# pangsu0613/TransCAR

Measured on AMD Instinct MI355X. Metric: nuScenes frames/sec (6-cam+radar, 900 queries): fusion decoder (Detr3DHead.forward + box decode), FPN features resident in HBM, higher is better.
Workload: dtype f32 (linear steps and attention core of the batched launches: f16x2 split operands, 3 v_mfma_f32_16x16x32_f16 products, fp32 accumulate; activations of the 32-row tiles held as two f16 planes; 4- / 8-row tiles: f32 MFMA)

## Files before the change

### include/transcar_hip.h

```cpp
#ifndef TRANSCAR_HIP_H
#define TRANSCAR_HIP_H

#include <stddef.h>

#ifdef __cplusplus
extern "C" {
#endif

#define TC_MAX_LEVELS 4
#define TC_MAX_LAYERS 8
#define TC_MAX_RADAR_LAYERS 3
#define TC_MAX_CAM_LOGITS 256
#define TC_RADAR_HEADS 8
#define TC_MAX_CLASSES 32
#define TC_BOX_DECODE_MAX_SCORES 12288
#define TC_BOX_DECODE_MAX_NUM 512
#define TC_BOX_DECODE_STREAM_MAX_SCORES (1 << 20)
#define TC_BOX_DECODE_STREAM_MAX_NUM 2048
#define TC_LSA_MAX_QUERIES 4096
#define TC_LSA_MAX_GT 512
#define TC_LSA_SMALL_MAX_QUERIES 1024
#define TC_LSA_SMALL_MAX_GT 128
#define TC_LSA_AUTO 0
#define TC_LSA_SMALL 1
// ... 127 lines not shown

int tc_refine_reference_fwd(const float* reg_out, int code_size, const float* ref,
                            float* new_ref, int M, tc_stream_t stream);

int tc_cam_sample_fuse_fwd(const tc_feats_nhwc* feats, int B, int Q, int C, int num_cams,
                           const float* lidar2img , const float* ref ,
                           const float* attn_logits ,
                           const float* pc_range , float img_h, float img_w,
                           float* out, unsigned char* vis_mask,
                           unsigned long long* pair_counter ,
                           tc_stream_t stream);

int tc_cam_sample_fuse_points_fwd(const tc_feats_nhwc* feats, int B, int Q, int C, int num_cams, int num_points,
                                  const float* lidar2img , const float* ref ,
                                  const float* attn_logits ,
                                  const float* pc_range , float img_h, float img_w,
                                  float* out, unsigned char* vis_mask,
                                  unsigned long long* pair_counter ,
                                  tc_stream_t stream);

size_t tc_cross_atten_workspace_bytes(int B, int Q, int C, int num_cams, int num_levels);
int tc_cross_atten_fwd(const tc_linear* attention_weights, const tc_linear* output_proj,
                       const tc_pos_encoder* position_encoder,
                       const tc_feats_nhwc* feats, int B, int Q, int C, int num_cams,
                       const float* query, const float* query_pos,
                       const float* lidar2img, const float* ref,
                       const float* pc_range , float img_h, float img_w,
                       float* out, void* workspace, size_t workspace_bytes,
                       tc_stream_t stream);
size_t tc_cross_atten_points_workspace_bytes(int B, int Q, int C, int num_cams, int num_levels, int num_points);
int tc_cross_atten_points_fwd(const tc_linear* attention_weights, const tc_linear* output_proj,
                              const tc_pos_encoder* position_encoder,
                              const tc_feats_nhwc* feats, int B, int Q, int C, int num_cams, int num_points,
                              const float* query, const float* query_pos,
                              const float* lidar2img, const float* ref,
                              const float* pc_range , float img_h, float img_w,
                              float* out, void* workspace, size_t workspace_bytes,
                              tc_stream_t stream);

size_t tc_self_attn_workspace_bytes(int B, int Q, int C);
int tc_self_attn_fwd(const tc_mha* w, const float* x, const float* pos, float* out,
                     int B, int Q, int C, int num_heads,
                     void* workspace, size_t workspace_bytes, tc_stream_t stream);

int tc_decoder_layer_tail_fwd(const tc_decoder_layer* layer, const tc_linear* next_in_proj,
                              const tc_feats_nhwc* feats, int B, int Q, int num_cams,
                              int code_size, const float* attn_o, const float* x_in,
                              const float* query_embedding, const float* lidar2img,
                              const float* ref_in, const float* pc_range ,
                              float img_h, float img_w, float* hs, float* ref_out,
                              float* qk, float* vt, int qpad,
                              int tile_rows , tc_stream_t stream);

int tc_sdpa_fwd(const float* q, const float* k, int ld, const float* vt, int ldt,
                float* out, int ldo, int B, int Q, int num_heads, tc_stream_t stream);
size_t tc_sdpa_f16x2_workspace_bytes(int B, int Q, int num_heads);
int tc_sdpa_fwd_f16x2(const float* qk, const float* vt, int ldt, float* out, int ldo, int B, int Q, int num_heads,
                      void* workspace, size_t workspace_bytes, tc_stream_t stream);
int tc_sdpa_fwd_hd(const float* q, const float* k, int ld, const float* vt, int ldt,
                   float* out, int ldo, int B, int Q, int num_heads, int head_dim, tc_stream_t stream);
int tc_sdpa_fwd_f16x2_hd(const float* qk, const float* vt, int ldt, float* out, int ldo, int B, int Q, int num_heads,
                         int head_dim, tc_stream_t stream);

size_t tc_radar_xattn_workspace_bytes(int B, int Q, int T, int C);
int tc_radar_gated_xattn_fwd(const tc_mha* w, const float* query, const float* centre_xy,
                             const float* box, int code_size,
                             const float* radar_feat, const float* radar_xy,
                             int B, int Q, int T, int C, int num_heads, int pad_mult,
                             float radius_min, float radius_max,
                             float* out, int* hit_counts,
                             void* workspace, size_t workspace_bytes, tc_stream_t stream);

int tc_radar_fusion_fwd(const tc_head_weights* packed_view, const float* hs_last,
                        const float* ref_last, const float* prev_box, const float* radar_tokens,
                        int B, int T, int pad_mult, int first_layer, int num_layers,
                        float* all_cls_scores, float* all_bbox_preds, int* hit_counts,
                        const tc_head_options* options, void* workspace, size_t workspace_bytes,
                        tc_stream_t stream);

int tc_radar_gate_selfcheck(int n_radii, unsigned long long seed, unsigned long long* mismatches,
                            tc_stream_t stream);

int tc_rowops_selfcheck(int n_blocks, unsigned long long seed, unsigned long long* mismatches, tc_stream_t stream);

size_t tc_box_decode_workspace_bytes(int B, int Q, int num_classes);
int tc_box_decode_topk(const float* cls_scores ,
                       const float* bbox_preds , int B, int Q,
                       int num_classes, int code_size, int max_num,
                       const float* post_center_range ,
                       float* boxes, float* scores, int* labels, unsigned char* valid,
                       void* workspace, size_t workspace_bytes, tc_stream_t stream);
int tc_box_decode_kept(const float* cls_scores, const float* bbox_preds, int B, int Q, int num_classes,
                       int code_size, int max_num, const float* post_center_range ,
                       float score_threshold, int use_threshold, int z_shift,
                       float* kept_boxes, float* kept_scores, long long* kept_labels, int* kept_count,
                       tc_stream_t stream);
int tc_box_decode_topk_path(const float* cls_scores, const float* bbox_preds, int B, int Q,
                            int num_classes, int code_size, int max_num,
                            const float* post_center_range ,
                            float* boxes, float* scores, int* labels, unsigned char* valid,
                            void* workspace, size_t workspace_bytes, tc_stream_t stream, int path);
int tc_box_decode_kept_path(const float* cls_scores, const float* bbox_preds, int B, int Q, int num_classes,
                            int code_size, int max_num, const float* post_center_range ,
                            float score_threshold, int use_threshold, int z_shift,
                            float* kept_boxes, float* kept_scores, long long* kept_labels, int* kept_count,
                            tc_stream_t stream, int path);

size_t tc_head_workspace_bytes(const tc_head_weights* w, int B, int T);
size_t tc_cam_pregather_workspace_bytes(const tc_head_weights* w, int B);
size_t tc_head_packed_bytes(const tc_head_weights* w);
int tc_head_pack_weights(const tc_head_weights* w, void* packed, size_t packed_bytes,
                         tc_head_weights* packed_view, tc_stream_t stream);
int tc_head_repack_trainable(const tc_head_weights* w, tc_head_weights* packed_view,
                             tc_stream_t stream);
int tc_head_repack_trainable_ex(const tc_head_weights* w, tc_head_weights* packed_view, int copies,
                                tc_stream_t stream);
int tc_head_forward(const tc_head_weights* w, const tc_head_weights* packed_view,
                    const tc_feats_nhwc* feats, int B,
                    const float* lidar2img , float img_h, float img_w,
                    const float* radar_tokens, int T, int pad_mult,
                    float* all_cls_scores, float* all_bbox_preds,
                    const tc_head_aux* aux ,
                    const tc_head_options* options ,
                    void* workspace, size_t workspace_bytes, tc_stream_t stream);

typedef struct {
  int abi_version;
  int num_levels, embed_dims, num_classes, code_size;
  float pc_range[6];
  tc_cls_branch cls[TC_MAX_LAYERS];
  tc_reg_branch reg[TC_MAX_LAYERS];
  size_t packed16_delta;
} tc_decoder_heads;
size_t tc_decoder_heads_packed_bytes(const tc_decoder_heads* w);
int tc_decoder_heads_pack(const tc_decoder_heads* w, void* packed, size_t packed_bytes,
                          tc_decoder_heads* packed_view, tc_stream_t stream);
int tc_decoder_outputs_fwd(const tc_decoder_heads* packed_view,
                           const float* inter_states     ,
                           const float* init_reference   ,
                           const float* inter_references ,
                           int B, int Q,
                           float* all_cls_scores ,
                           float* all_bbox_preds ,
                           const tc_head_options* options , tc_stream_t stream);



int tc_linear_gated_fwd(const float* x, const float* w, const float* b, const float* res,
                        const int* row_gate, float* y, int M, int K, int N, tc_stream_t stream);

int tc_linear_bwd_data(const float* dy, const float* y_relu, const int* row_gate,
                       const float* w, const float* x_relu, float* dx, int M, int K, int N,
                       float alpha, int accumulate, tc_stream_t stream);
int tc_linear_bwd_weight(const float* x, const float* dy, const float* y_relu,
                         const int* row_gate, float* dw, float* db, int M, int K, int N,
                         float alpha, tc_stream_t stream);

int tc_add_layernorm_bwd(const float* a, const float* b, const float* gamma, const float* dy,
                         const float* y_relu, float* dz, float* dgamma, float* dbeta, int M,
                         int C, tc_stream_t stream);

int tc_radar_reference_l1(const float* ref, const float* pc_range , float* centre_xy,
                          float* add_ref, int M, tc_stream_t stream);

int tc_box_add_ref_fwd(const float* reg_out, int code_size, const float* ref_xy, int ld_xy,
                       const float* ref_z, int ld_z, float* box, int M, tc_stream_t stream);
// ... 102 lines not shown
```

### transcar_amd/_lib.py

```python
import ctypes as C
import os

import torch

_HERE = os.path.dirname(os.path.abspath(__file__))
LIB_PATH = os.environ.get('TRANSCAR_HIP_LIB') or os.path.join(_HERE, 'lib', 'libtranscar_hip.so')

TC_MAX_LEVELS = 4
TC_MAX_LAYERS = 8
TC_MAX_RADAR_LAYERS = 3
TC_ABI_VERSION = 13

c_fp = C.c_void_p


class TransCARHipError(RuntimeError):
    pass


TC_MAX_CAM_LOGITS = 256


def check_num_points(num_points, num_cams, num_levels):
    if int(num_points) < 1 or num_cams * num_levels * int(num_points) > TC_MAX_CAM_LOGITS:
# ... 127 lines not shown
                ('num_points', C.c_int)]


class tc_decoder_heads(C.Structure):
    _fields_ = [('abi_version', C.c_int), ('num_levels', C.c_int), ('embed_dims', C.c_int),
                ('num_classes', C.c_int), ('code_size', C.c_int),
                ('pc_range', C.c_float * 6),
                ('cls', tc_cls_branch * TC_MAX_LAYERS), ('reg', tc_reg_branch * TC_MAX_LAYERS),
                ('packed16_delta', C.c_size_t)]


class tc_feats_nhwc(C.Structure):
    _fields_ = [('num_levels', C.c_int),
                ('data', c_fp * TC_MAX_LEVELS),
                ('H', C.c_int * TC_MAX_LEVELS),
                ('W', C.c_int * TC_MAX_LEVELS)]


class tc_head_aux(C.Structure):
    _fields_ = [('inter_states', c_fp), ('init_reference', c_fp),
                ('inter_references', c_fp), ('radar_hit_counts', c_fp),
                ('last_box', c_fp), ('sample_pairs', c_fp)]


class tc_head_options(C.Structure):
    _fields_ = [('chain_tile_rows', C.c_int), ('unfused', C.c_int),
                ('last_level_cls_only', C.c_int), ('reuse_radar_kv', C.c_int),
                ('decoder_dropout_p', C.c_float), ('radar_row_order', C.c_int),
                ('dropout_seed', C.c_ulonglong), ('phase', C.c_int), ('matrix_path', C.c_int),
                ('dropout_seed_stride', C.c_ulonglong), ('range_status', c_fp), ('cam_pregather', C.c_int),
                ('cam_pregather_ws', c_fp), ('cam_pregather_bytes', C.c_size_t)]


TC_MATRIX_AUTO, TC_MATRIX_F32, TC_MATRIX_F16X2 = 0, 1, 2


_P = C.POINTER
_i, _f, _sz, _vp = C.c_int, C.c_float, C.c_size_t, C.c_void_p

SIGNATURES = {
    'tc_abi_version': (_i, []),
    'tc_last_error': (C.c_char_p, []),
    'tc_chain_tile_rows': (_i, [_i, _i, _i]),
    'tc_device_count': (_i, []),
    'tc_nchw_to_nhwc': (_i, [_vp, _vp, _i, _i, _i, _i, _vp]),
    'tc_nchw_to_nhwc_levels': (_i, [_P(_vp), _P(_vp), _i, _i, _i, _P(_i), _P(_i), _vp]),
    'tc_radar_build_tokens': (_i, [_vp, _vp, _P(_i), _i, _P(C.c_double), _P(C.c_double),
                                   _P(C.c_double), _vp, _i, _vp, _vp]),
    'tc_radar_build_tokens_batch': (_i, [_vp, _vp, _vp, _i, _i, _vp, _i, _vp, _vp]),
    'tc_linear_fwd': (_i, [_vp, _vp, _vp, _vp, _vp, _vp, _i, _i, _i, _i, _vp]),
    'tc_add_layernorm_fwd': (_i, [_vp, _vp, _vp, _vp, _vp, _i, _i, _i, _vp]),
    'tc_refine_reference_fwd': (_i, [_vp, _i, _vp, _vp, _i, _vp]),
    'tc_cam_sample_fuse_fwd': (_i, [_P(tc_feats_nhwc), _i, _i, _i, _i, _vp,
                                    _vp, _vp, _P(_f), _f, _f, _vp, _vp, _vp,
                                    _vp]),
    'tc_cam_sample_fuse_points_fwd': (_i, [_P(tc_feats_nhwc), _i, _i, _i, _i, _i,
                                           _vp, _vp, _vp, _P(_f), _f, _f, _vp,
                                           _vp, _vp, _vp]),
    'tc_cross_atten_workspace_bytes': (_sz, [_i, _i, _i, _i, _i]),
    'tc_cross_atten_points_workspace_bytes': (_sz, [_i, _i, _i, _i, _i, _i]),
    'tc_cross_atten_points_fwd': (_i, [_P(tc_linear), _P(tc_linear),
                                       _P(tc_pos_encoder), _P(tc_feats_nhwc),
                                       _i, _i, _i, _i, _i, _vp, _vp, _vp, _vp,
                                       _P(_f), _f, _f, _vp, _vp, _sz, _vp]),
    'tc_cross_atten_fwd': (_i, [_P(tc_linear), _P(tc_linear),
                                _P(tc_pos_encoder), _P(tc_feats_nhwc), _i, _i,
                                _i, _i, _vp, _vp, _vp, _vp, _P(_f), _f, _f,
                                _vp, _vp, _sz, _vp]),
    'tc_self_attn_workspace_bytes': (_sz, [_i, _i, _i]),
    'tc_self_attn_fwd': (_i, [_P(tc_mha), _vp, _vp, _vp, _i, _i, _i, _i, _vp,
                              _sz, _vp]),
    'tc_decoder_layer_tail_fwd': (_i, [_P(tc_decoder_layer), _P(tc_linear),
                                       _P(tc_feats_nhwc), _i, _i, _i, _i, _vp,
                                       _vp, _vp, _vp, _vp, _P(_f), _f, _f, _vp,
                                       _vp, _vp, _vp, _i, _i, _vp]),
    'tc_sdpa_fwd': (_i, [_vp, _vp, _i, _vp, _i, _vp, _i, _i, _i, _i, _vp]),
    'tc_sdpa_f16x2_workspace_bytes': (_sz, [_i, _i, _i]),
    'tc_sdpa_fwd_f16x2': (_i, [_vp, _vp, _i, _vp, _i, _i, _i, _i, _vp, _sz, _vp]),
    'tc_sdpa_fwd_hd': (_i, [_vp, _vp, _i, _vp, _i, _vp, _i, _i, _i, _i, _i, _vp]),
    'tc_sdpa_fwd_f16x2_hd': (_i, [_vp, _vp, _i, _vp, _i, _i, _i, _i, _i, _vp]),
    'tc_radar_xattn_workspace_bytes': (_sz, [_i, _i, _i, _i]),
    'tc_radar_gate_selfcheck': (_i, [_i, C.c_ulonglong, _vp, _vp]),
    'tc_rowops_selfcheck': (_i, [_i, C.c_ulonglong, _vp, _vp]),
    'tc_radar_gated_xattn_fwd': (_i, [_P(tc_mha), _vp, _vp, _vp, _i, _vp, _vp,
                                      _i, _i, _i, _i, _i, _i, _f, _f, _vp,
                                      _vp, _vp, _sz, _vp]),
    'tc_radar_fusion_fwd': (_i, [_P(tc_head_weights), _vp, _vp, _vp, _vp, _i, _i, _i, _i, _i,
                                 _vp, _vp, _vp, _P(tc_head_options), _vp, _sz, _vp]),
    'tc_box_decode_workspace_bytes': (_sz, [_i, _i, _i]),
    'tc_box_decode_topk': (_i, [_vp, _vp, _i, _i, _i, _i, _i, _P(_f), _vp,
                                _vp, _vp, _vp, _vp, _sz, _vp]),
    'tc_box_decode_kept': (_i, [_vp, _vp, _i, _i, _i, _i, _i, _P(_f), _f, _i, _i, _vp, _vp, _vp, _vp, _vp]),
    'tc_box_decode_topk_path': (_i, [_vp, _vp, _i, _i, _i, _i, _i, _P(_f), _vp,
                                     _vp, _vp, _vp, _vp, _sz, _vp, _i]),
    'tc_box_decode_kept_path': (_i, [_vp, _vp, _i, _i, _i, _i, _i, _P(_f), _f, _i, _i, _vp, _vp, _vp, _vp, _vp, _i]),
    'tc_head_workspace_bytes': (_sz, [_P(tc_head_weights), _i, _i]),
    'tc_cam_pregather_workspace_bytes': (_sz, [_P(tc_head_weights), _i]),
    'tc_head_packed_bytes': (_sz, [_P(tc_head_weights)]),
    'tc_head_pack_weights': (_i, [_P(tc_head_weights), _vp, _sz,
                                  _P(tc_head_weights), _vp]),
    'tc_head_repack_trainable': (_i, [_P(tc_head_weights), _P(tc_head_weights), _vp]),
    'tc_head_forward': (_i, [_P(tc_head_weights), _P(tc_head_weights),
                             _P(tc_feats_nhwc), _i, _vp,
                             _f, _f, _vp, _i, _i, _vp, _vp, _P(tc_head_aux),
                             _P(tc_head_options), _vp, _sz, _vp]),
    'tc_decoder_heads_packed_bytes': (_sz, [_P(tc_decoder_heads)]),
    'tc_decoder_heads_pack': (_i, [_P(tc_decoder_heads), _vp, _sz, _P(tc_decoder_heads), _vp]),
    'tc_decoder_outputs_fwd': (_i, [_P(tc_decoder_heads), _vp, _vp, _vp, _i, _i, _vp, _vp,
                                    _P(tc_head_options), _vp]),
    'tc_linear_gated_fwd': (_i, [_vp, _vp, _vp, _vp, _vp, _vp, _i, _i, _i, _vp]),
    'tc_linear_bwd_data': (_i, [_vp, _vp, _vp, _vp, _vp, _vp, _i, _i, _i, _f,
                                _i, _vp]),
    'tc_linear_bwd_weight': (_i, [_vp, _vp, _vp, _vp, _vp, _vp, _i, _i, _i, _f,
                                  _vp]),
    'tc_add_layernorm_bwd': (_i, [_vp, _vp, _vp, _vp, _vp, _vp, _vp, _vp, _i,
                                  _i, _vp]),
    'tc_radar_reference_l1': (_i, [_vp, _P(_f), _vp, _vp, _i, _vp]),
    'tc_box_add_ref_fwd': (_i, [_vp, _i, _vp, _i, _vp, _i, _vp, _i, _vp]),
    'tc_box_add_ref_bwd': (_i, [_vp, _i, _vp, _i, _vp]),
    'tc_radar_attn_core_fwd': (_i, [_vp, _f, _vp, _vp, _i, _vp, _i, _vp, _i,
                                    _i, _i, _i, _i, _i, _i, _f, _f, _vp, _vp,
                                    _f, C.c_ulonglong, _i, _vp]),
    'tc_dropout': (_i, [_vp, _i, _i, _f, C.c_ulonglong, _i, _vp, _vp]),
    'tc_radar_attn_core_bwd': (_i, [_vp, _f, _vp, _vp, _i, _vp, _i, _vp, _i,
                                    _i, _i, _i, _i, _i, _i, _f, _f, _vp, _vp,
                                    _vp, _vp, _f, C.c_ulonglong, _i, _vp]),
    'tc_radar_train_tape_bytes': (_sz, [_P(tc_head_weights), _i, _i]),
    'tc_radar_train_fwd': (_i, [_P(tc_head_weights), _vp, _vp, _vp, _vp, _i, _i,
                                _i, _vp, _vp, _vp, _sz, _f, C.c_ulonglong, _vp]),
    'tc_radar_train_fwd_fused': (_i, [_P(tc_head_weights), _vp, _vp, _vp, _vp, _i, _i,
                                      _i, _vp, _vp, _vp, _sz, _f, C.c_ulonglong, _vp]),
    'tc_head_repack_trainable_ex': (_i, [_P(tc_head_weights), _P(tc_head_weights), _i, _vp]),
    'tc_radar_train_bwd': (_i, [_P(tc_head_weights), _P(tc_head_weights), _vp,
                                _vp, _vp, _i, _i, _i, _vp, _vp, _vp, _vp, _sz,
                                _f, C.c_ulonglong, _vp]),
    'tc_radar_train_bwd_workspace_bytes': (_sz, [_P(tc_head_weights), _i, _i]),
    'tc_radar_train_bwd_fused': (_i, [_P(tc_head_weights), _P(tc_head_weights), _vp,
                                      _vp, _vp, _i, _i, _i, _vp, _vp, _vp, _vp, _sz, _vp, _sz,
                                      _f, C.c_ulonglong, _vp, _vp, _vp]),
    'tc_radar_train_bwd_fused_ex': (_i, [_P(tc_head_weights), _P(tc_head_weights), _vp,
                                         _vp, _vp, _i, _i, _i, _vp, _vp, _vp, _vp, _sz, _vp, _sz,
                                         _f, C.c_ulonglong, _vp, _vp, _i, _vp]),
    'tc_radar_train_bwd_fused_det': (_i, [_P(tc_head_weights), _P(tc_head_weights), _vp,
                                          _vp, _vp, _i, _i, _i, _vp, _vp, _vp, _vp, _sz, _vp, _sz,
                                          _f, C.c_ulonglong, _vp, _vp, _i, _vp, _sz, _vp, _sz, _vp]),
    'tc_radar_train_bwd_weights': (_i, [_P(tc_head_weights), _P(tc_head_weights), _vp, _vp, _i, _i, _vp, _sz, _vp, _sz,
                                        _i, _vp]),
    'tc_radar_train_repack': (_i, [_P(tc_head_weights), _P(tc_head_weights), _vp, _sz, _i, _i, _vp]),
    'tc_dropout_mask': (_i, [_f, C.c_ulonglong, _i, _sz, _vp, _vp]),
    'tc_normalize_bbox': (_i, [_vp, _i, _vp, _vp]),
    'tc_match_cost': (_i, [_vp, _vp, _i, _i, _i, _i, _i, _vp, _vp, _vp, _i, _f, _f,
                           _f, _f, _f, _vp, _vp]),
    'tc_detr_loss_fwd_bwd': (_i, [_vp, _vp, _i, _i, _i, _i, _i, _vp, _vp, _i, _vp,
                                  _vp, _vp, _f, _f, _f, _f, _vp, _vp, _vp, _vp]),
    'tc_detr_loss_fwd_bwd_counts': (_i, [_vp, _vp, _i, _i, _i, _i, _i, _vp, _vp, _i, _vp,
                                         _vp, _vp, _f, _f, _f, _f, _vp, _vp, _vp, _vp]),
    'tc_lsa_assign': (_i, [_vp, _vp, _i, _i, _i, _i, _vp, _vp, _vp, _vp]),
    'tc_lsa_assign_ex': (_i, [_vp, _vp, _i, _i, _i, _i, _vp, _vp, _vp, _vp, _vp]),
    'tc_lsa_workspace_bytes': (_sz, [_i, _i, _i, _i]),
    'tc_lsa_assign_ws': (_i, [_vp, _vp, _i, _i, _i, _i, _vp, _vp, _vp, _vp, _vp, _sz, _i, _vp]),
    'tc_sq_norm': (_i, [_vp, _sz, _vp, _vp]),
    'tc_adamw_step': (_i, [_vp, _vp, _vp, _vp, _sz, _f, _f, _f, _f, _f, _i, _f,
                           _f, _vp, _vp]),
}

_lib = None
# ... 57 lines not shown
```

### transcar_amd/csrc/chain.hip

```cpp
#include <stdlib.h>
#include <string.h>

#include <type_traits>

#include "kernels.hpp"
#ifdef TC_CHAIN_STAMPS
__device__ long long g_cam_stamps[4][8];
#define CAM_STAMP(slot)                                                                        \
  do {                                                                                         \
    if (blockIdx.x == 100 && (threadIdx.x & 63) == 0)                                          \
      g_cam_stamps[(threadIdx.x >> 6) & 3][(slot)] = __builtin_amdgcn_s_memtime();             \
  } while (0)
#endif
#include "rowdev.hpp"
#define TC_ONCE_LD(p) ldg4_stream(p)
#ifdef TC_CHAIN_DUMP
__device__ float* g_chain_dump;
__device__ long long g_chain_dump_floats;
#endif

namespace tc {

namespace {

constexpr int CH_NW = 4;
constexpr int CH_NT = CH_NW * 64;
constexpr int CH_NW_MAX = 8;
constexpr int nw_of(int R) { return R == 32 ? 8 : 4; }
constexpr int LD5 = 516;
constexpr int LD2 = 260;
constexpr int LDL = 36;

struct StepRes {
  const float* p0; const float* p1; const float* p2; const float* p3;
  float* gd; float* gt;
  int K, N, gld, gmod;
  short kind, src, src2, dst, res, act, flags, sync, rep, si;
  int src_off, src2_off;
  int pad_;
};
struct EpiRec {
  float* gd; float* gt;
  int dst_off, res_off, dst_ld, res_ld;
  int gld, act, flags, N;
  int has_bias, woff;
  int drop_site;
  int pad1;
};
struct PreRec { const float* first; int nidx; int pad; };
template <int NW> struct StepAllT { StepRes r; EpiRec e; PreRec p[NW]; };
using StepAll = StepAllT<CH_NW>;
static_assert(sizeof(StepAllT<CH_NW>) % 16 == 0 && sizeof(StepAllT<CH_NW_MAX>) % 16 == 0, "records are copied 16 bytes at a time");
template <int N, int NW = CH_NW> struct Recs { StepAllT<NW> s[N]; };

constexpr int HM_WORDS = 8;
static_assert(HM_WORDS * 8 <= LDL * 4 && (LDL * 4) % 8 == 0, "hit masks live in a row of the logit buffer");
template <int R, int NREC>
struct ChainLds {
  StepAllT<nw_of(R)> recs[NREC];
  float unit[4][R][LD2];
  float l[R][LDL];
  float box[R][12];
  float cen[R][4];
  int gate[R];
  int rowg[R];
};
static_assert(LD5 * 1 <= 2 * LD2, "the 512-wide tile must fit two units");

#ifdef TC_CHAIN_STAMPS
#define CHAIN_DBG(v) (v)
#else
#define CHAIN_DBG(v) 0
#endif

#define MFMA44(a, b, c, grp) __builtin_amdgcn_mfma_f32_4x4x1f32((a), (b), (c), 4, (grp), 0)

enum Buf : short { B_NONE = -1, B_A = 0 , B_X , B_U1, B_U2, B_U3, B_L };
enum Kind : short {
  K_END = 0, K_LOAD, K_LINEAR, K_LN, K_POSENC, K_SAMPLE, K_REFUPD, K_TOKENS, K_RADAR_ATTN, K_BOXADD, K_RADAR_GATE,
  K_NARROW,
  K_NOP,
  K_LOADG,
  K_MASKCOPY,
  K_LN_BWD,
  K_ATTN_BWD,
  K_BOXSIG
};
enum NSpecial : short { N_LOGITS = -1, N_CODE = -2, N_CLS = -3 };
enum Flags : short {
  F_GATE = 1,
  F_SCALEQ = 2,
  F_WOFF = 4,
  F_LN_RELU = 8,
  F_SKIP_NONEXT = 16,
  F_WAVE1 = 32,
  F_NOT_W0 = 64,
  F_LN_XP = 128,
  F_IFHIT = 256,
  F_GPRE = 512,
  F_CMASK = 1024,
  F_CMASK_SCALE = 2048,
  F_CARRY = 4096,
  F_NOT_LAYER0 = 8192,
  F_PRESYNC = 16384
};
enum GSel : short {
  G_NONE = -1, G_HS = 0, G_QK, G_VT, G_INITREF, G_ATTN_O, G_XIN, G_POS, G_CLS, G_KV0, G_KV1, G_KV2,
  G_QF, G_RFEAT, G_COUNT
};

struct StepDesc {
  short kind, wp, wp2, K, N, src, src2, dst, res, act, flags, gsel, gtsel, sync;
};
constexpr StepDesc PROG_DECODER_T[] = {
    {K_LOAD, 0, 0, 0, 0, B_NONE, B_NONE, B_U1, B_NONE, 0, 0, G_ATTN_O, G_NONE, 0},
    {K_LOAD, 0, 0, 0, 0, B_NONE, B_NONE, B_X, B_NONE, 0, 0, G_XIN, G_NONE, 1},
    {K_LINEAR, 1, -1, 256, 256, B_U1, B_NONE, B_U2, B_X, 0, 0, G_NONE, G_NONE, 1},
    {K_LN, 2, -1, 0, 0, B_U2, B_NONE, B_X, B_U1, 0, F_LN_XP, G_NONE, G_NONE, 1},
    {K_LINEAR, 3, -1, 256, N_LOGITS, B_U1, B_NONE, B_L, B_NONE, 0, 0, G_NONE, G_NONE, 0},
    {K_POSENC, 5, 6, 0, 0, B_NONE, B_NONE, B_U2, B_NONE, 0, F_NOT_W0, G_NONE, G_NONE, 1},
    {K_SAMPLE, 0, 0, 0, 0, B_L, B_NONE, B_U3, B_NONE, 0, 0, G_NONE, G_NONE, 1},
    {K_LINEAR, 7, -1, 256, 256, B_U2, B_NONE, B_U1, B_NONE, 0, 0, G_NONE, G_NONE, 1},
    {K_LINEAR, 4, -1, 256, 256, B_U3, B_NONE, B_U2, B_X, 0, 0, G_NONE, G_NONE, 1},
    {K_LN, 9, 8, 0, 0, B_U2, B_U1, B_X, B_NONE, 0, 0, G_NONE, G_NONE, 1},
    {K_LINEAR, 10, -1, 256, 512, B_X, B_NONE, B_A, B_NONE, 1, 0, G_NONE, G_NONE, 1},
    {K_LINEAR, 11, -1, 512, 256, B_A, B_NONE, B_U3, B_X, 0, 0, G_NONE, G_NONE, 1},
    {K_LN, 12, -1, 0, 0, B_U3, B_NONE, B_X, B_U1, 0, F_LN_XP, G_HS, G_NONE, 1},
    {K_LINEAR, 13, -1, 256, 256, B_X, B_NONE, B_U2, B_NONE, 1, 0, G_NONE, G_NONE, 0},
    {K_LINEAR, 16, -1, 256, 512, B_U1, B_NONE, B_NONE, B_NONE, 0, F_SCALEQ | F_SKIP_NONEXT, G_QK, G_NONE, 0},
    {K_LINEAR, 16, -1, 256, 256, B_X, B_NONE, B_NONE, B_NONE, 0, F_WOFF | F_SKIP_NONEXT, G_NONE, G_VT, 1},
    {K_LINEAR, 14, -1, 256, 256, B_U2, B_NONE, B_U3, B_NONE, 1, 0, G_NONE, G_NONE, 0},
    {K_NARROW, 15, -1, 256, N_CODE, B_U3, B_U1, B_L, B_NONE, 0, F_PRESYNC, G_NONE, G_NONE, 1},
    {K_REFUPD, 0, 0, 0, 0, B_L, B_NONE, B_NONE, B_NONE, 0, 0, G_NONE, G_NONE, 0},
    {K_END, 0, 0, 0, 0, 0, 0, 0, 0, 0, 0, 0, 0, 0}};
constexpr StepDesc PROG_DECODER_L0_T[] = {
    {K_LOAD, 0, 0, 0, 0, B_NONE, B_NONE, B_U1, B_NONE, 0, 0, G_ATTN_O, G_NONE, 0},
    {K_LOAD, 0, 0, 0, 0, B_NONE, B_NONE, B_U2, B_NONE, 0, 0, G_KV1, G_NONE, 0},
    {K_LOAD, 0, 0, 0, 0, B_NONE, B_NONE, B_X, B_NONE, 0, 0, G_XIN, G_NONE, 1},
    {K_LINEAR, 3, -1, 256, N_LOGITS, B_U1, B_NONE, B_L, B_NONE, 0, 0, G_NONE, G_NONE, 0},
    {K_POSENC, 5, 6, 0, 0, B_NONE, B_NONE, B_U3, B_NONE, 0, F_NOT_W0, G_NONE, G_NONE, 1},
    {K_SAMPLE, 0, 0, 0, 0, B_L, B_NONE, B_U3, B_NONE, 0, 0, G_NONE, G_NONE, 1},
    {K_LINEAR, 4, -1, 256, 256, B_U3, B_NONE, B_U1, B_X, 0, 0, G_NONE, G_NONE, 1},
    {K_LN, 9, 8, 0, 0, B_U1, B_U2, B_X, B_NONE, 0, 0, G_NONE, G_NONE, 1},
    {K_LINEAR, 10, -1, 256, 512, B_X, B_NONE, B_A, B_NONE, 1, 0, G_NONE, G_NONE, 1},
    {K_LINEAR, 11, -1, 512, 256, B_A, B_NONE, B_U3, B_X, 0, 0, G_NONE, G_NONE, 1},
    {K_LN, 12, -1, 0, 0, B_U3, B_NONE, B_X, B_U1, 0, F_LN_XP, G_HS, G_NONE, 1},
    {K_LINEAR, 13, -1, 256, 256, B_X, B_NONE, B_U2, B_NONE, 1, 0, G_NONE, G_NONE, 0},
    {K_LINEAR, 16, -1, 256, 512, B_U1, B_NONE, B_NONE, B_NONE, 0, F_SCALEQ | F_SKIP_NONEXT, G_QK, G_NONE, 0},
    {K_LINEAR, 16, -1, 256, 256, B_X, B_NONE, B_NONE, B_NONE, 0, F_WOFF | F_SKIP_NONEXT, G_NONE, G_VT, 1},
    {K_LINEAR, 14, -1, 256, 256, B_U2, B_NONE, B_U3, B_NONE, 1, 0, G_NONE, G_NONE, 0},
    {K_NARROW, 15, -1, 256, N_CODE, B_U3, B_U1, B_L, B_NONE, 0, F_PRESYNC, G_NONE, G_NONE, 1},
    {K_REFUPD, 0, 0, 0, 0, B_L, B_NONE, B_NONE, B_NONE, 0, 0, G_NONE, G_NONE, 0},
    {K_END, 0, 0, 0, 0, 0, 0, 0, 0, 0, 0, 0, 0, 0}};
constexpr StepDesc PROG_DECODER_L0GEN_T[] = {
    {K_LOAD, 0, 0, 0, 0, B_NONE, B_NONE, B_U1, B_NONE, 0, 0, G_ATTN_O, G_NONE, 0},
    {K_LOAD, 0, 0, 0, 0, B_NONE, B_NONE, B_X, B_NONE, 0, 0, G_XIN, G_NONE, 1},
    {K_LINEAR, 1, -1, 256, 256, B_U1, B_NONE, B_U2, B_X, 0, 0, G_NONE, G_NONE, 1},
    {K_LN, 2, -1, 0, 0, B_U2, B_NONE, B_X, B_U1, 0, F_LN_XP, G_KV0, G_NONE, 1},
    {K_POSENC, 5, 6, 0, 0, B_NONE, B_NONE, B_U2, B_NONE, 0, F_NOT_W0, G_NONE, G_NONE, 1},
    {K_LINEAR, 7, -1, 256, 256, B_U2, B_NONE, B_U1, B_NONE, 0, 0, G_KV1, G_NONE, 1},
    {K_END, 0, 0, 0, 0, 0, 0, 0, 0, 0, 0, 0, 0, 0}};
static_assert(sizeof(PROG_DECODER_L0_T) <= sizeof(PROG_DECODER_T) && sizeof(PROG_DECODER_L0GEN_T) <= sizeof(PROG_DECODER_T),
              "the layer-0 sequences fit the decoder program's records");
constexpr StepDesc PROG_PROLOGUE_T[] = {
    {K_LOAD, 0, 0, 0, 0, B_NONE, B_NONE, B_U1, B_NONE, 0, 0, G_POS, G_NONE, 0},
    {K_LOAD, 0, 0, 0, 0, B_NONE, B_NONE, B_X, B_NONE, 0, 0, G_XIN, G_NONE, 1},
    {K_LINEAR, 0, -1, 256, 3, B_U1, B_NONE, B_NONE, B_NONE, 2, 0, G_INITREF, G_NONE, 0},
    {K_LINEAR, 16, -1, 256, 512, B_X, B_U1, B_NONE, B_NONE, 0, F_SCALEQ, G_QK, G_NONE, 0},
    {K_LINEAR, 16, -1, 256, 256, B_X, B_NONE, B_NONE, B_NONE, 0, F_WOFF, G_NONE, G_VT, 0},
    {K_END, 0, 0, 0, 0, 0, 0, 0, 0, 0, 0, 0, 0, 0}};
constexpr StepDesc PROG_RADAR_ENC_T[] = {
    {K_TOKENS, 0, 0, 0, 0, B_NONE, B_NONE, B_A, B_NONE, 0, 0, G_NONE, G_NONE, 1},
    {K_POSENC, 0, 1, 0, 0, B_A, B_NONE, B_U3, B_NONE, 0, 0, G_NONE, G_NONE, 0},
    {K_LINEAR, 4, -1, 36, 64, B_A, B_NONE, B_X, B_NONE, 1, 0, G_NONE, G_NONE, 1},
    {K_LINEAR, 2, -1, 256, 256, B_U3, B_NONE, B_U1, B_NONE, 0, 0, G_NONE, G_NONE, 0},
    {K_LINEAR, 5, -1, 64, 128, B_X, B_NONE, B_U2, B_NONE, 1, 0, G_NONE, G_NONE, 1},
    {K_LINEAR, 6, -1, 128, 256, B_U2, B_NONE, B_X, B_NONE, 1, 0, G_NONE, G_NONE, 1},
    {K_LN, 3, -1, 0, 0, B_U1, B_NONE, B_U2, B_X, 0, F_LN_RELU, G_NONE, G_NONE, 1},
    {K_LINEAR, 7, -1, 256, 512, B_U2, B_NONE, B_NONE, B_NONE, 0, 0, G_KV0, G_NONE, 0},
    {K_LINEAR, 8, -1, 256, 512, B_U2, B_NONE, B_NONE, B_NONE, 0, 0, G_KV1, G_NONE, 0},
    {K_LINEAR, 9, -1, 256, 512, B_U2, B_NONE, B_NONE, B_NONE, 0, 0, G_KV2, G_NONE, 0},
    {K_END, 0, 0, 0, 0, 0, 0, 0, 0, 0, 0, 0, 0, 0}};
constexpr StepDesc PROG_RADAR_ENC_A_T[] = {
    {K_TOKENS, 0, 0, 0, 0, B_NONE, B_NONE, B_A, B_NONE, 0, 0, G_NONE, G_NONE, 1},
    {K_POSENC, 0, 1, 0, 0, B_A, B_NONE, B_U3, B_NONE, 0, 0, G_NONE, G_NONE, 0},
    {K_LINEAR, 4, -1, 36, 64, B_A, B_NONE, B_X, B_NONE, 1, 0, G_NONE, G_NONE, 1},
    {K_LINEAR, 2, -1, 256, 256, B_U3, B_NONE, B_U1, B_NONE, 0, 0, G_NONE, G_NONE, 0},
    {K_LINEAR, 5, -1, 64, 128, B_X, B_NONE, B_U2, B_NONE, 1, 0, G_NONE, G_NONE, 1},
    {K_LINEAR, 6, -1, 128, 256, B_U2, B_NONE, B_X, B_NONE, 1, 0, G_NONE, G_NONE, 1},
    {K_LN, 3, -1, 0, 0, B_U1, B_NONE, B_U2, B_X, 0, F_LN_RELU, G_RFEAT, G_NONE, 1},
    {K_LINEAR, 7, -1, 256, 512, B_U2, B_NONE, B_NONE, B_NONE, 0, 0, G_KV0, G_NONE, 0},
    {K_END, 0, 0, 0, 0, 0, 0, 0, 0, 0, 0, 0, 0, 0}};
constexpr StepDesc PROG_RADAR_ENC_B_T[] = {
    {K_LOAD, 0, 0, 0, 0, B_NONE, B_NONE, B_X, B_NONE, 0, 0, G_RFEAT, G_NONE, 1},
    {K_LINEAR, 8, -1, 256, 512, B_X, B_NONE, B_NONE, B_NONE, 0, 0, G_KV1, G_NONE, 0},
    {K_LINEAR, 9, -1, 256, 512, B_X, B_NONE, B_NONE, B_NONE, 0, 0, G_KV2, G_NONE, 0},
    {K_END, 0, 0, 0, 0, 0, 0, 0, 0, 0, 0, 0, 0, 0}};
constexpr StepDesc PROG_RADAR_LAYER_T[] = {
    {K_RADAR_GATE, 0, 0, 0, 0, B_NONE, B_NONE, B_NONE, B_NONE, 0, 0, G_NONE, G_NONE, 1},
    {K_LINEAR, 0, -1, 256, 256, B_X, B_NONE, B_U1, B_NONE, 0, F_SCALEQ | F_IFHIT, G_NONE, G_NONE, 1},
    {K_RADAR_ATTN, 0, 0, 0, 0, B_U1, B_NONE, B_U2, B_NONE, 0, F_IFHIT, G_NONE, G_NONE, 1},
    {K_LINEAR, 1, -1, 256, 256, B_U2, B_NONE, B_U3, B_X, 0, F_GATE | F_IFHIT, G_NONE, G_NONE, 1},
    {K_LN, 2, -1, 0, 0, B_U3, B_NONE, B_X, B_NONE, 0, 0, G_NONE, G_NONE, 1},
    {K_LINEAR, 3, -1, 256, 512, B_X, B_NONE, B_A, B_NONE, 1, 0, G_NONE, G_NONE, 1},
    {K_LINEAR, 4, -1, 512, 256, B_A, B_NONE, B_U3, B_X, 0, 0, G_NONE, G_NONE, 1},
    {K_LN, 5, -1, 0, 0, B_U3, B_NONE, B_X, B_NONE, 0, 0, G_NONE, G_NONE, 1},
    {K_LINEAR, 6, -1, 256, 256, B_X, B_NONE, B_U1, B_NONE, 0, 0, G_NONE, G_NONE, 0},
    {K_LINEAR, 11, -1, 256, 256, B_X, B_NONE, B_U2, B_NONE, 1, 0, G_NONE, G_NONE, 1},
    {K_LN, 7, -1, 0, 0, B_U1, B_NONE, B_U1, B_NONE, 0, F_LN_RELU, G_NONE, G_NONE, 0},
    {K_LINEAR, 12, -1, 256, 256, B_U2, B_NONE, B_U3, B_NONE, 1, 0, G_NONE, G_NONE, 1},
    {K_LINEAR, 8, -1, 256, 256, B_U1, B_NONE, B_U2, B_NONE, 0, 0, G_NONE, G_NONE, 1},
    {K_LN, 9, -1, 0, 0, B_U2, B_NONE, B_U2, B_NONE, 0, F_LN_RELU, G_NONE, G_NONE, 0},
    {K_NARROW, 13, -1, 256, N_CODE, B_U3, B_U1, B_L, B_NONE, 0, F_PRESYNC, G_NONE, G_NONE, 0},
    {K_NARROW, 10, -1, 256, N_CLS, B_U2, B_U1, B_NONE, B_NONE, 0, F_PRESYNC, G_CLS, G_NONE, 1},
    {K_BOXADD, 0, 0, 0, 0, B_L, B_NONE, B_NONE, B_NONE, 0, 0, G_NONE, G_NONE, 1},
    {K_END, 0, 0, 0, 0, 0, 0, 0, 0, 0, 0, 0, 0, 0}};

constexpr StepDesc PROG_DECODER_HEADS_T[] = {
    {K_LOAD, 0, 0, 0, 0, B_NONE, B_NONE, B_X, B_NONE, 0, 0, G_HS, G_NONE, 1},
    {K_LINEAR, 0, -1, 256, 256, B_X, B_NONE, B_U1, B_NONE, 0, 0, G_NONE, G_NONE, 0},
    {K_LINEAR, 5, -1, 256, 256, B_X, B_NONE, B_U2, B_NONE, 1, 0, G_NONE, G_NONE, 1},
    {K_LN, 1, -1, 0, 0, B_U1, B_NONE, B_U1, B_NONE, 0, F_LN_RELU, G_NONE, G_NONE, 0},
    {K_LINEAR, 6, -1, 256, 256, B_U2, B_NONE, B_U3, B_NONE, 1, 0, G_NONE, G_NONE, 1},
    {K_LINEAR, 2, -1, 256, 256, B_U1, B_NONE, B_U2, B_NONE, 0, 0, G_NONE, G_NONE, 1},
    {K_LN, 3, -1, 0, 0, B_U2, B_NONE, B_U2, B_NONE, 0, F_LN_RELU, G_NONE, G_NONE, 0},
    {K_NARROW, 7, -1, 256, N_CODE, B_U3, B_U1, B_L, B_NONE, 0, F_PRESYNC, G_NONE, G_NONE, 0},
    {K_NARROW, 4, -1, 256, N_CLS, B_U2, B_U1, B_NONE, B_NONE, 0, F_PRESYNC, G_CLS, G_NONE, 0},
    {K_NARROW, 4, -1, 256, N_CLS, B_U2, B_U1, B_NONE, B_NONE, 1, F_PRESYNC, G_CLS, G_NONE, 1},
    {K_BOXSIG, 0, 0, 0, 0, B_L, B_NONE, B_NONE, B_NONE, 0, 0, G_NONE, G_NONE, 0},
    {K_END, 0, 0, 0, 0, 0, 0, 0, 0, 0, 0, 0, 0, 0}};

constexpr StepDesc PROG_RADAR_BWD_T[] = {
    {K_LOADG, 0, 0, 0, N_CODE, B_NONE, B_NONE, B_U1, B_NONE, 0, F_CARRY, G_NONE, G_NONE, 1},
    {K_LINEAR, 13, -1, N_CODE, 256, B_U1, B_NONE, B_U2, B_NONE, 0, F_CMASK, G_NONE, G_NONE, 1},
    {K_LINEAR, 12, -1, 256, 256, B_U2, B_NONE, B_U1, B_NONE, 0, F_CMASK, G_NONE, G_NONE, 1},
    {K_LINEAR, 11, -1, 256, 256, B_U1, B_NONE, B_U3, B_X, 0, 0, G_NONE, G_NONE, 1},
    {K_LOADG, 0, 0, 0, N_CLS, B_NONE, B_NONE, B_U1, B_NONE, 0, 0, G_NONE, G_NONE, 1},
    {K_LINEAR, 10, -1, N_CLS, 256, B_U1, B_NONE, B_U2, B_NONE, 0, 0, G_NONE, G_NONE, 1},
    {K_LN_BWD, 9, -1, 0, 0, B_U2, B_NONE, B_U1, B_X, 0, F_LN_RELU, G_NONE, G_NONE, 1},
    {K_LINEAR, 8, -1, 256, 256, B_U1, B_NONE, B_U2, B_NONE, 0, 0, G_NONE, G_NONE, 1},
    {K_LN_BWD, 7, -1, 0, 0, B_U2, B_NONE, B_U1, B_X, 0, F_LN_RELU, G_NONE, G_NONE, 1},
    {K_LINEAR, 6, -1, 256, 256, B_U1, B_NONE, B_X, B_U3, 0, 0, G_NONE, G_NONE, 1},
    {K_LN_BWD, 5, -1, 0, 0, B_X, B_NONE, B_X, B_U1, 0, 0, G_NONE, G_NONE, 1},
    {K_MASKCOPY, 0, 0, 3, 0, B_X, B_NONE, B_U3, B_NONE, 0, 0, G_NONE, G_NONE, 1},
    {K_LINEAR, 4, -1, 256, 512, B_U3, B_NONE, B_A, B_NONE, 0, F_CMASK | F_CMASK_SCALE, G_NONE, G_NONE, 1},
    {K_LINEAR, 3, -1, 512, 256, B_A, B_NONE, B_U3, B_X, 0, 0, G_NONE, G_NONE, 1},
    {K_LN_BWD, 2, -1, 0, 0, B_U3, B_NONE, B_X, B_U1, 0, 0, G_NONE, G_NONE, 1},
    {K_MASKCOPY, 0, 0, 1, 0, B_X, B_NONE, B_U1, B_NONE, 0, F_GATE, G_NONE, G_NONE, 1},
    {K_LINEAR, 1, -1, 256, 256, B_U1, B_NONE, B_U2, B_NONE, 0, 0, G_NONE, G_NONE, 1},
    {K_ATTN_BWD, 0, 0, 0, 0, B_U2, B_NONE, B_U1, B_NONE, 0, 0, G_NONE, G_NONE, 1},
    {K_LINEAR, 0, -1, 256, 256, B_U1, B_NONE, B_X, B_X, 0, F_NOT_LAYER0, G_NONE, G_NONE, 1},
    {K_END, 0, 0, 0, 0, 0, 0, 0, 0, 0, 0, 0, 0, 0}};
enum DSel : short { D_NONE = -1, D_DBOX = 0, D_DT1, D_DT0, D_DC2, D_DC0, D_DFF, D_DH, D_DPROJ, D_DQP, D_DCLS, D_COUNT };
constexpr short BWD_STORE[19] = {D_DBOX, D_DT1, D_DT0, D_NONE, D_DCLS, D_NONE, D_DC2, D_NONE, D_DC0, D_NONE, D_NONE, D_DFF,
                                 D_DH, D_NONE, D_NONE, D_DPROJ, D_NONE, D_DQP, D_NONE};
enum Program : int { PROG_PROLOGUE = 0, PROG_DECODER, PROG_RADAR_ENC, PROG_RADAR, PROG_RADAR_ENC_A, PROG_RADAR_ENC_B,
                     PROG_RADAR_TRAIN, PROG_RADAR_ENC_TRAIN, PROG_RADAR_BWD, PROG_DECODER_HEADS };
constexpr bool prog_is_radar(int p) { return p == PROG_RADAR || p == PROG_RADAR_TRAIN; }
constexpr bool prog_is_enc_full(int p) { return p == PROG_RADAR_ENC || p == PROG_RADAR_ENC_TRAIN; }
enum TSel : short { T_NONE = -1, T_QP = 0, T_AO, T_X1, T_X2, T_H, T_FF, T_X3, T_C0, T_C1, T_C2, T_C3, T_T0, T_T1, T_TREG,
                    E_U0, E_U1, E_U2, E_POS, E_F0, E_F1, E_F2, E_MEM, T_COUNT };
constexpr short RADAR_TAPE[17] = {T_NONE, T_QP, T_AO, T_X1, T_X2, T_H, T_FF, T_X3, T_C0, T_T0, T_C1, T_T1, T_C2, T_C3,
                                  T_TREG, T_NONE, T_NONE};
constexpr short ENC_TAPE[10] = {T_NONE, E_U1, E_F0, E_U2, E_F1, E_F2, E_MEM, T_NONE, T_NONE, T_NONE};
constexpr short ENC_TAPE2[10] = {T_NONE, E_U0, T_NONE, T_NONE, T_NONE, T_NONE, E_POS, T_NONE, T_NONE, T_NONE};
constexpr short BWD_TAPE[19] = {T_NONE, T_T1, T_T0, T_NONE, T_NONE, T_NONE, T_C2, T_NONE, T_C0, T_NONE, T_X2, T_NONE,
                                T_H, T_NONE, T_X1, T_NONE, T_NONE, T_NONE, T_NONE};
constexpr short BWD_TAPE2[19] = {T_NONE, T_NONE, T_NONE, T_NONE, T_NONE, T_NONE, T_C3, T_NONE, T_C1, T_NONE, T_FF, T_NONE,
                                 T_NONE, T_NONE, T_NONE, T_NONE, T_NONE, T_NONE, T_NONE};

constexpr int MAX_PAIRS = 48;
constexpr int RADAR_PAIRS = 14;

struct ChainDev {
  int program, M, Q, code, ncls, nlogits, has_next, nlayers;
  int total, early_n;
  float* g[G_COUNT]; int g_ld[G_COUNT]; int g_mod[G_COUNT];
  float qscale; int qpad;
  DropK drop;
  int dbg;
  int tile_rows;
  int matrix_path;
  int last_cls_only;
  const float* ref_in; int ref_mod; float* ref_out; float* box_m;
  CamK cam; unsigned long long* pair_counter;
  const float* pre; const int* premask;
  const float* tokens; int RI, T, pad_mult;
  const float* ref_last; const float* box_in;
  int cen_from_box;
  float rmin[TC_MAX_RADAR_LAYERS], rmax[TC_MAX_RADAR_LAYERS];
  float* all_box; int* hits;
  const int* row_perm;
  float* tape[T_COUNT]; size_t tape_stride; size_t hits_stride;
  DropK rdrop;
  const float* bwd_cxy[TC_MAX_RADAR_LAYERS]; int bwd_ldc[TC_MAX_RADAR_LAYERS];
  const float* bwd_box[TC_MAX_RADAR_LAYERS];
  int* range_status;
  const float* loss_vals;
  float* loss_out;
  const DetAcc* detp;
};
struct ChainK : ChainDev {
  tc_linear pairs[MAX_PAIRS];
  tc_linear gpairs[MAX_PAIRS];
  float* dy[D_COUNT]; size_t dy_stride = 0;
  const float* d_cls = nullptr; const float* d_box = nullptr;
  float* dkv[TC_MAX_RADAR_LAYERS] = {nullptr, nullptr, nullptr};
  size_t w16_delta = 0;
  int npoints = 1;
  int refine = 1;
  int l0_seq = 0;
};

inline bool generic_xattn(const ChainK& k) { return k.npoints > 1 || k.cam.num_levels < 4; }

constexpr int table_steps(int prog) {
  return (prog == PROG_DECODER ? (int)(sizeof(PROG_DECODER_T) / sizeof(StepDesc))
          : prog == PROG_PROLOGUE ? (int)(sizeof(PROG_PROLOGUE_T) / sizeof(StepDesc))
          : prog_is_enc_full(prog) ? (int)(sizeof(PROG_RADAR_ENC_T) / sizeof(StepDesc))
          : prog == PROG_RADAR_ENC_A ? (int)(sizeof(PROG_RADAR_ENC_A_T) / sizeof(StepDesc))
          : prog == PROG_RADAR_ENC_B ? (int)(sizeof(PROG_RADAR_ENC_B_T) / sizeof(StepDesc))
          : prog == PROG_RADAR_BWD ? (int)(sizeof(PROG_RADAR_BWD_T) / sizeof(StepDesc))
          : prog == PROG_DECODER_HEADS ? (int)(sizeof(PROG_DECODER_HEADS_T) / sizeof(StepDesc))
                                     : (int)(sizeof(PROG_RADAR_LAYER_T) / sizeof(StepDesc))) - 1;
}
constexpr int rec_cap(int prog) { return table_steps(prog) * ((prog_is_radar(prog) || prog == PROG_RADAR_BWD) ? TC_MAX_RADAR_LAYERS : 1); }
static_assert(sizeof(BWD_STORE) / sizeof(short) == table_steps(PROG_RADAR_BWD), "backward maps follow the step table");
static_assert(sizeof(RADAR_TAPE) / sizeof(short) == table_steps(PROG_RADAR) && sizeof(ENC_TAPE) / sizeof(short) == table_steps(PROG_RADAR_ENC),
              "tape maps follow the step tables");
inline const StepDesc* prog_table(int prog) {
  return prog == PROG_DECODER ? PROG_DECODER_T
         : prog == PROG_PROLOGUE ? PROG_PROLOGUE_T
         : prog_is_enc_full(prog) ? PROG_RADAR_ENC_T
         : prog == PROG_RADAR_ENC_A ? PROG_RADAR_ENC_A_T
         : prog == PROG_RADAR_ENC_B ? PROG_RADAR_ENC_B_T
         : prog == PROG_RADAR_BWD ? PROG_RADAR_BWD_T
         : prog == PROG_DECODER_HEADS ? PROG_DECODER_HEADS_T : PROG_RADAR_LAYER_T;
}

struct LinSpec {
  const float* W; const float* bias; int K, N;
  const float* src; int src_ld;
  const float* src2; int src2_ld;
  float* dst; int dst_ld;
  const float* res; int res_ld;
  const int* gate;
  int act; float scale; int scale_cols;
  float* gdst; int gdst_ld;
  float* gt; int gt_ld, gt_rpb;
  int m0, M;
  int woff;
  int dbg;
  int sub_on;
  int drop_site;
  unsigned long long drop_seed; unsigned drop_thr; float drop_scale;
  unsigned long long drop_stride; int drop_q;
  const int* rowg;
  int gpre;
  const float* cmask; float cscale;
  int dst_pl, res_pl;
  int* range_flag;
};

constexpr int KB = 64;
struct WBuf { float4 b[16]; };

#ifdef TC_CHAIN_STAMPS
__device__ long long g_chain_sub[CH_NW_MAX][64];
__device__ int g_sub_step;
#define SUB_STAMP(slot)                                                                       \
  do {                                                                                        \
    if (blockIdx.x == 100 && (threadIdx.x & 63) == 0 && s.sub_on && (slot) < 64)              \
      g_chain_sub[threadIdx.x >> 6][(slot)] = __builtin_amdgcn_s_memtime();                   \
  } while (0)
#else
#define SUB_STAMP(slot) do {} while (0)
#endif

__device__ __forceinline__ void wload(WBuf& wb, const float* w, int nq) {
#pragma unroll
  for (int i = 0; i < 16; ++i)
    wb.b[i] = i < nq ? ld4(w + i * 256) : make_float4(0.f, 0.f, 0.f, 0.f);
}

template <int NG>
struct Acc { f32x4 v[NG][2]; };

template <int NG>
__device__ __forceinline__ void acc_zero(Acc<NG>& a) {
#pragma unroll
  for (int g = 0; g < NG; ++g) { a.v[g][0] = f32x4{0.f, 0.f, 0.f, 0.f}; a.v[g][1] = f32x4{0.f, 0.f, 0.f, 0.f}; }
}

template <int NG, bool PF, int J>
struct ItemSteps {
  static __device__ __forceinline__ void run(Acc<NG>& acc, const WBuf& wb, const float4* ar, WBuf& nx,
                                             const float* np) {
    if (PF) nx.b[J] = ld4(np + J * 256);
    __builtin_amdgcn_sched_barrier(0);
#pragma unroll
    for (int g = 0; g < NG; ++g) {
      acc.v[g][0] = MFMA44(ar[g].x, wb.b[J].x, acc.v[g][0], J);
      acc.v[g][1] = MFMA44(ar[g].y, wb.b[J].y, acc.v[g][1], J);
      acc.v[g][0] = MFMA44(ar[g].z, wb.b[J].z, acc.v[g][0], J);
      acc.v[g][1] = MFMA44(ar[g].w, wb.b[J].w, acc.v[g][1], J);
    }
    __builtin_amdgcn_sched_barrier(0);
    ItemSteps<NG, PF, J + 1>::run(acc, wb, ar, nx, np);
  }
};
template <int NG, bool PF>
struct ItemSteps<NG, PF, 16> {
  static __device__ __forceinline__ void run(Acc<NG>&, const WBuf&, const float4*, WBuf&, const float*) {}
};

template <int NG, bool PF>
__device__ __forceinline__ void wcompute(Acc<NG>& acc, const WBuf& wb, const float4* ar, WBuf& nx,
                                         const float* np) {
  ItemSteps<NG, PF, 0>::run(acc, wb, ar, nx, np);
}

template <int NG, bool DROP>
__device__ __forceinline__ void lin_epilogue(const LinSpec& s, int tile, const Acc<NG>& acc, int lane, float bv) {
  const int col = tile * 64 + lane;
  if (col >= s.N) return;
  const float sc = (col < s.scale_cols) ? s.scale : 1.0f;
  const float bias = s.bias != nullptr ? bv : 0.0f;
  float y[NG][4];
#pragma unroll
  for (int g = 0; g < NG; ++g)
#pragma unroll
    for (int i = 0; i < 4; ++i) y[g][i] = ((acc.v[g][0][i] + acc.v[g][1][i]) + bias) * sc;
  if (s.act == 1) {
#pragma unroll
    for (int g = 0; g < NG; ++g)
#pragma unroll
      for (int i = 0; i < 4; ++i) y[g][i] = relu_(y[g][i]);
  } else if (s.act == 2) {
#pragma unroll
    for (int g = 0; g < NG; ++g)
#pragma unroll
      for (int i = 0; i < 4; ++i) y[g][i] = sigmoidf_(y[g][i]);
  }
  if constexpr (DROP) {
// ... 294 lines not shown
      asm volatile("" : "+s"(tile), "+s"(sidx));
      if (!(CHAIN_DBG(s.dbg) & 1)) {
        const LinSpec e = make_spec(sidx);
        lin_epilogue16<DROP>(e, tile * 64, acc.v, lane, bvl);
      }
    }
    wcur = np; tt = nt; kb = nk;
    __builtin_amdgcn_sched_barrier(0);
  }
  return next_first != nullptr;
}

typedef _Float16 f16x8 __attribute__((ext_vector_type(8)));
typedef _Float16 f16x2 __attribute__((ext_vector_type(2)));
#define MFMA16H(a, b, c) __builtin_amdgcn_mfma_f32_16x16x32_f16(__builtin_bit_cast(f16x8, (a)), __builtin_bit_cast(f16x8, (b)), (c), 0, 0, 0)
constexpr float H_ACT_SCALE = 1.0f / 64.0f;
constexpr float H_LO_SCALE = 2048.0f;
struct Acc16H { f32x4 hi[4]; f32x4 lo[4]; };

__device__ __forceinline__ unsigned pk_h2(float a, float b) {
  const f16x2 v = {(_Float16)a, (_Float16)b};
  return __builtin_bit_cast(unsigned, v);
}
__device__ __forceinline__ void split_t2(float t0, float t1, unsigned& hi, unsigned& lo) {
  hi = pk_h2(t0, t1);
  asm("" : "+v"(hi));
  float m1 = -1.0f;
  asm("" : "+s"(m1));
  const f16x2 h = __builtin_bit_cast(f16x2, hi);
  const float r0 = __builtin_fmaf((float)h[0], m1, t0), r1 = __builtin_fmaf((float)h[1], m1, t1);
  const f16x2 l = {(_Float16)__builtin_fmaf(r0, H_LO_SCALE, 0.0f), (_Float16)__builtin_fmaf(r1, H_LO_SCALE, 0.0f)};
  lo = __builtin_bit_cast(unsigned, l);
}
__device__ __forceinline__ void split_h(const float4& a, const float4& b, float4& p1, float4& p2) {
  const float x[8] = {a.x, a.y, a.z, a.w, b.x, b.y, b.z, b.w};
  unsigned q1[4], q2[4];
#pragma unroll
  for (int i = 0; i < 4; ++i) split_t2(x[2 * i] * H_ACT_SCALE, x[2 * i + 1] * H_ACT_SCALE, q1[i], q2[i]);
  p1 = make_float4(__uint_as_float(q1[0]), __uint_as_float(q1[1]), __uint_as_float(q1[2]), __uint_as_float(q1[3]));
  p2 = make_float4(__uint_as_float(q2[0]), __uint_as_float(q2[1]), __uint_as_float(q2[2]), __uint_as_float(q2[3]));
}

template <bool PL>
__device__ __forceinline__ float4 act_ld4(const float* row, int col) {
  if constexpr (!PL) {
    return *reinterpret_cast<const float4*>(row + col);
  } else {
    const char* p = reinterpret_cast<const char*>(row) + (col >> 3) * 32 + (col & 7) * 2;
    const uint2 h = *reinterpret_cast<const uint2*>(p), l = *reinterpret_cast<const uint2*>(p + 16);
    const f16x2 h0 = __builtin_bit_cast(f16x2, h.x), h1 = __builtin_bit_cast(f16x2, h.y);
    const f16x2 l0 = __builtin_bit_cast(f16x2, l.x), l1 = __builtin_bit_cast(f16x2, l.y);
    constexpr float US = 1.0f / H_ACT_SCALE, UL = 1.0f / H_LO_SCALE;
    return make_float4(fmaf((float)l0[0], UL, (float)h0[0]) * US, fmaf((float)l0[1], UL, (float)h0[1]) * US,
                       fmaf((float)l1[0], UL, (float)h1[0]) * US, fmaf((float)l1[1], UL, (float)h1[1]) * US);
  }
}
template <bool PL>
__device__ __forceinline__ void act_st4(float* row, int col, const float4& v) {
  if constexpr (!PL) {
    *reinterpret_cast<float4*>(row + col) = v;
  } else {
    const float t0 = v.x * H_ACT_SCALE, t1 = v.y * H_ACT_SCALE, t2 = v.z * H_ACT_SCALE, t3 = v.w * H_ACT_SCALE;
    uint2 h, l;
    split_t2(t0, t1, h.x, l.x);
    split_t2(t2, t3, h.y, l.y);
    char* p = reinterpret_cast<char*>(row) + (col >> 3) * 32 + (col & 7) * 2;
    *reinterpret_cast<uint2*>(p) = h;
    *reinterpret_cast<uint2*>(p + 16) = l;
  }
}

template <bool PL>
__device__ __forceinline__ float act_ld1(const float* row, int col) {
  if constexpr (!PL) {
    return row[col];
  } else {
    const char* p = reinterpret_cast<const char*>(row) + (col >> 3) * 32 + (col & 7) * 2;
    const _Float16 h = *reinterpret_cast<const _Float16*>(p), l = *reinterpret_cast<const _Float16*>(p + 16);
    constexpr float US = 1.0f / H_ACT_SCALE, UL = 1.0f / H_LO_SCALE;
    return fmaf((float)l, UL, (float)h) * US;
  }
}

struct Acc32H;
template <bool DROP>
__device__ __forceinline__ void lin_epilogue32(const LinSpec& s, int colbase, const f32x4 (&thi)[4], const f32x4 (&tlo)[4], int lane,
                                               const float4 (&bias4)[2]) {
  const int c = lane & 15, g = lane >> 4;
  const int colb = colbase + 4 * g;
  constexpr float US = 1.0f / H_ACT_SCALE;
  uint2 rh[4], rl[4];
  float4 rf[4];
  const bool res_planes = s.res != nullptr && s.res_pl, res_f32 = s.res != nullptr && !s.res_pl;
  if (res_planes) {
#pragma unroll
    for (int v = 0; v < 4; ++v) {
      const int col = colb + 16 * (v & 1), row = 16 * (v >> 1) + c;
      const char* p = reinterpret_cast<const char*>(s.res + row * s.res_ld) + (col >> 3) * 32 + (col & 7) * 2;
      rh[v] = *reinterpret_cast<const uint2*>(p); rl[v] = *reinterpret_cast<const uint2*>(p + 16);
    }
  } else if (res_f32) {
#pragma unroll
    for (int v = 0; v < 4; ++v)
      rf[v] = *reinterpret_cast<const float4*>(s.res + (16 * (v >> 1) + c) * s.res_ld + colb + 16 * (v & 1));
  }
  float t[4][4];
#pragma unroll
  for (int v = 0; v < 4; ++v)
#pragma unroll
    for (int i = 0; i < 4; ++i) t[v][i] = fmaf(tlo[v][i], 1.0f / H_LO_SCALE, thi[v][i]);
  if (s.bias != nullptr) {
#pragma unroll
    for (int v = 0; v < 4; ++v) {
      const float4 b4 = bias4[v & 1];
      t[v][0] = fmaf(b4.x, H_ACT_SCALE, t[v][0]); t[v][1] = fmaf(b4.y, H_ACT_SCALE, t[v][1]);
      t[v][2] = fmaf(b4.z, H_ACT_SCALE, t[v][2]); t[v][3] = fmaf(b4.w, H_ACT_SCALE, t[v][3]);
    }
  }
  if (colbase < s.scale_cols) {
#pragma unroll
    for (int v = 0; v < 4; ++v)
#pragma unroll
      for (int i = 0; i < 4; ++i) t[v][i] *= s.scale;
  }
  if (s.range_flag != nullptr) {
    bool bad = false;
#pragma unroll
    for (int v = 0; v < 4; ++v)
#pragma unroll
      for (int i = 0; i < 4; ++i) bad |= !(fabsf(t[v][i]) <= 3.0e38f * H_ACT_SCALE);
    if (__builtin_amdgcn_ballot_w64(bad) != 0 && lane == 0) atomicOr(s.range_flag, 1);
  }
  if (s.act == 1) {
#pragma unroll
    for (int v = 0; v < 4; ++v)
#pragma unroll
      for (int i = 0; i < 4; ++i) t[v][i] = relu_(t[v][i]);
  } else if (s.act == 2) {
#pragma unroll
    for (int v = 0; v < 4; ++v)
#pragma unroll
      for (int i = 0; i < 4; ++i) t[v][i] = sigmoidf_(t[v][i] * US) * H_ACT_SCALE;
  }
  if (s.gate != nullptr) {
#pragma unroll
    for (int rg = 0; rg < 2; ++rg)
      if (s.gate[16 * rg + c] == 0) {
#pragma unroll
        for (int jj = 0; jj < 2; ++jj)
#pragma unroll
          for (int i = 0; i < 4; ++i) t[2 * rg + jj][i] = 0.0f;
      }
  }
  if (DROP) {
    if (s.drop_site != 0) {
#pragma unroll
      for (int rg = 0; rg < 2; ++rg) {
        unsigned row = (unsigned)(s.m0 + 16 * rg + c);
        unsigned long long seed = s.drop_seed;
        if (s.drop_q > 0) { const unsigned b = row / (unsigned)s.drop_q; row -= b * (unsigned)s.drop_q; seed += b * s.drop_stride; }
#pragma unroll
        for (int jj = 0; jj < 2; ++jj) {
          const unsigned m = drop_keep4(seed, (unsigned)(s.drop_site - 1), row * (unsigned)s.N + (unsigned)(colb + 16 * jj), s.drop_thr);
#pragma unroll
          for (int i = 0; i < 4; ++i) t[2 * rg + jj][i] = ((m >> i) & 1u) ? t[2 * rg + jj][i] * s.drop_scale : 0.0f;
        }
      }
    }
  }
  if (res_planes) {
#pragma unroll
    for (int v = 0; v < 4; ++v) {
      const f16x2 h0 = __builtin_bit_cast(f16x2, rh[v].x), h1 = __builtin_bit_cast(f16x2, rh[v].y);
      const f16x2 l0 = __builtin_bit_cast(f16x2, rl[v].x), l1 = __builtin_bit_cast(f16x2, rl[v].y);
      t[v][0] += fmaf((float)l0[0], 1.0f / H_LO_SCALE, (float)h0[0]); t[v][1] += fmaf((float)l0[1], 1.0f / H_LO_SCALE, (float)h0[1]);
      t[v][2] += fmaf((float)l1[0], 1.0f / H_LO_SCALE, (float)h1[0]); t[v][3] += fmaf((float)l1[1], 1.0f / H_LO_SCALE, (float)h1[1]);
    }
  } else if (res_f32) {
#pragma unroll
    for (int v = 0; v < 4; ++v) {
      t[v][0] = fmaf(rf[v].x, H_ACT_SCALE, t[v][0]); t[v][1] = fmaf(rf[v].y, H_ACT_SCALE, t[v][1]);
      t[v][2] = fmaf(rf[v].z, H_ACT_SCALE, t[v][2]); t[v][3] = fmaf(rf[v].w, H_ACT_SCALE, t[v][3]);
    }
  }
  if (s.dst != nullptr) {
    if (s.dst_pl) {
#pragma unroll
      for (int v = 0; v < 4; ++v) {
        const int col = colb + 16 * (v & 1), rloc = 16 * (v >> 1) + c;
        uint2 h, l;
        split_t2(t[v][0], t[v][1], h.x, l.x);
        split_t2(t[v][2], t[v][3], h.y, l.y);
        char* p = reinterpret_cast<char*>(s.dst + rloc * s.dst_ld) + (col >> 3) * 32 + (col & 7) * 2;
        *reinterpret_cast<uint2*>(p) = h;
        *reinterpret_cast<uint2*>(p + 16) = l;
      }
    } else {
#pragma unroll
      for (int v = 0; v < 4; ++v)
        *reinterpret_cast<float4*>(s.dst + (16 * (v >> 1) + c) * s.dst_ld + colb + 16 * (v & 1)) =
            make_float4(t[v][0] * US, t[v][1] * US, t[v][2] * US, t[v][3] * US);
    }
  }
  if (s.gdst != nullptr || s.gt != nullptr) {
    const bool vec = (s.gdst_ld & 3) == 0;
#pragma unroll
    for (int v = 0; v < 4; ++v) {
      const int col = colb + 16 * (v & 1), rloc = 16 * (v >> 1) + c;
      if (s.m0 + rloc >= s.M) continue;
      const float4 y4 = make_float4(t[v][0] * US, t[v][1] * US, t[v][2] * US, t[v][3] * US);
      if (s.gdst != nullptr) {
        const int grow = s.rowg != nullptr ? s.rowg[rloc] : s.m0 + rloc;
        float* gp = s.gdst + (size_t)grow * s.gdst_ld + col;
        if (vec) st4(gp, y4);
        else { stg1(gp, y4.x); stg1(gp + 1, y4.y); stg1(gp + 2, y4.z); stg1(gp + 3, y4.w); }
      }
      if (s.gt != nullptr) {
        const int row = s.m0 + rloc;
        const int bb = row / s.gt_rpb, q = row - bb * s.gt_rpb;
        float* tp = s.gt + ((size_t)bb * s.N + col) * s.gt_ld + q;
        stg1(tp, y4.x); stg1(tp + s.gt_ld, y4.y); stg1(tp + 2 * (size_t)s.gt_ld, y4.z); stg1(tp + 3 * (size_t)s.gt_ld, y4.w);
      }
    }
  }
}

template <int J, int BUF>
struct ItemSteps16H {
  static __device__ __forceinline__ void run(Acc16H& acc, WBuf& wb, const float4& x1, const float4& x2, const float* np,
                                             unsigned lo) {
    constexpr int C0 = 8 * BUF + 2 * J, N0 = 8 * (1 - BUF) + 2 * J;
    acc.lo[J] = MFMA16H(wb.b[C0 + 1], x1, acc.lo[J]);
    acc.lo[J] = MFMA16H(wb.b[C0], x2, acc.lo[J]);
    acc.hi[J] = MFMA16H(wb.b[C0], x1, acc.hi[J]);
    __builtin_amdgcn_sched_barrier(0);
    wb.b[N0] = ld4(np + (size_t)(lo + (2 * J) * 256u));
    wb.b[N0 + 1] = ld4(np + (size_t)(lo + (2 * J + 1) * 256u));
    __builtin_amdgcn_sched_barrier(0);
    ItemSteps16H<J + 1, BUF>::run(acc, wb, x1, x2, np, lo);
  }
};
template <int BUF>
struct ItemSteps16H<4, BUF> {
  static __device__ __forceinline__ void run(Acc16H&, WBuf&, const float4&, const float4&, const float*, unsigned) {}
};

template <bool DROP, typename SpecFn>
__device__ __forceinline__ bool linear_step16h(const LinSpec& s, WBuf& w0, bool preloaded, const float* next_first,
                                               SpecFn make_spec, int step_idx) {
  const int lane = threadIdx.x & 63;
  const int wave = (__builtin_amdgcn_readfirstlane(threadIdx.x >> 6) - s.woff) & (CH_NW - 1);
  const int ntiles = (s.N + 63) >> 6;
  const int kpad = (s.K + 63) & ~63;
  const int nhalf = kpad / 32;
  const int my_tiles = wave < ntiles ? (ntiles - wave + CH_NW - 1) / CH_NW : 0;
  const int nitems = my_tiles * nhalf;
  const float* arow = s.src + (lane & 15) * s.src_ld + 8 * (lane >> 4);
  const float* wbase = s.W + (size_t)wave * 64 * kpad;
  const unsigned lo = 4u * lane;
  const size_t tile_stride = (size_t)CH_NW * 64 * kpad;
  Acc16H acc;
  float bvl = 0.f;
  SUB_STAMP(1);
  if (CHAIN_DBG(s.dbg) & 32) return false;
  if (!preloaded) {
// ... 5 lines not shown
  __builtin_amdgcn_s_waitcnt(0x0F70);
  int tt = 0, kh = 0;
  const float* wcur = wbase;
#pragma unroll 1
  for (int it = 0; it < nitems; it += 2) {
    {
      if (kh == 0) {
#pragma unroll
        for (int j = 0; j < 4; ++j) { acc.hi[j] = f32x4{0.f, 0.f, 0.f, 0.f}; acc.lo[j] = f32x4{0.f, 0.f, 0.f, 0.f}; }
        const float* bsrc = s.bias != nullptr ? s.bias : s.W;
        bvl = ldg1(bsrc + min((wave + tt * CH_NW) * 64 + lane, s.N - 1));
      }
      float4 x1, x2;
      split_h(*reinterpret_cast<const float4*>(arow + kh * 32), *reinterpret_cast<const float4*>(arow + kh * 32 + 4), x1, x2);
      ItemSteps16H<0, 0>::run(acc, w0, x1, x2, wcur + 8 * 256, lo);
      wcur += 8 * 256; ++kh;
      __builtin_amdgcn_sched_barrier(0);
    }
    {
      const float* np = wcur;
      int nt = tt, nk = kh;
      if (++nk == nhalf) { nk = 0; ++nt; np = wbase + (size_t)nt * tile_stride; }
      else np += 8 * 256;
      const bool last = it + 2 >= nitems;
      const float* nload = last ? (next_first != nullptr ? next_first : wbase) : np;
      float4 x1, x2;
      split_h(*reinterpret_cast<const float4*>(arow + kh * 32), *reinterpret_cast<const float4*>(arow + kh * 32 + 4), x1, x2);
      ItemSteps16H<0, 1>::run(acc, w0, x1, x2, nload, lo);
      if (kh == nhalf - 1) {
        int tile = wave + tt * CH_NW;
        int sidx = step_idx;
        asm volatile("" : "+s"(tile), "+s"(sidx));
        if (!(CHAIN_DBG(s.dbg) & 1)) {
          Acc16 y;
#pragma unroll
          for (int j = 0; j < 4; ++j)
#pragma unroll
            for (int i = 0; i < 4; ++i)
              y.v[j][i] = fmaf(acc.lo[j][i], 1.0f / (H_LO_SCALE * H_ACT_SCALE), acc.hi[j][i] * (1.0f / H_ACT_SCALE));
          const LinSpec e = make_spec(sidx);
          lin_epilogue16<DROP>(e, tile * 64, y.v, lane, bvl);
        }
      }
      wcur = np; tt = nt; kh = nk;
      __builtin_amdgcn_sched_barrier(0);
    }
  }
  return next_first != nullptr;
}


struct Acc32H { f32x4 hi[2][2]; f32x4 lo[2][2]; };

template <int BUF>
__device__ __forceinline__ void item32h(Acc32H& acc, WBuf& wb, const float* arow0, const float* arow1, int koff,
                                        const float* np, unsigned lo) {
  constexpr int C = 8 * BUF, N = 8 * (1 - BUF);
  float4 x1[2][2], x2[2][2];
#pragma unroll
  for (int kk = 0; kk < 2; ++kk) {
    x1[kk][0] = *reinterpret_cast<const float4*>(arow0 + koff + 32 * kk); x2[kk][0] = *reinterpret_cast<const float4*>(arow0 + koff + 32 * kk + 4);
    x1[kk][1] = *reinterpret_cast<const float4*>(arow1 + koff + 32 * kk); x2[kk][1] = *reinterpret_cast<const float4*>(arow1 + koff + 32 * kk + 4);
  }
  __builtin_amdgcn_sched_barrier(0);
#pragma unroll
  for (int kk = 0; kk < 2; ++kk) {
#pragma unroll
    for (int jj = 0; jj < 2; ++jj) {
      const int f = 4 * kk + 2 * jj;
#pragma unroll
      for (int rg = 0; rg < 2; ++rg) {
        acc.lo[rg][jj] = MFMA16H(wb.b[C + f + 1], x1[kk][rg], acc.lo[rg][jj]);
        acc.lo[rg][jj] = MFMA16H(wb.b[C + f], x2[kk][rg], acc.lo[rg][jj]);
        acc.hi[rg][jj] = MFMA16H(wb.b[C + f], x1[kk][rg], acc.hi[rg][jj]);
      }
      __builtin_amdgcn_sched_barrier(0);
      wb.b[N + f] = ld4(np + (size_t)(lo + (8 * kk + 2 * jj) * 256u));
      wb.b[N + f + 1] = ld4(np + (size_t)(lo + (8 * kk + 2 * jj + 1) * 256u));
      __builtin_amdgcn_sched_barrier(0);
    }
  }
}

template <bool DROP, bool NB = false, typename SpecFn>
__device__ __forceinline__ bool linear_step32h(const LinSpec& s, WBuf& w0, bool preloaded, const float* next_first,
                                               SpecFn make_spec, int step_idx) {
  constexpr int NW = 8;
  const int lane = threadIdx.x & 63;
  const int wave = (__builtin_amdgcn_readfirstlane(threadIdx.x >> 6) - s.woff) & (NW - 1);
  const int ntiles = (s.N + 31) >> 5;
  const int kpad = (s.K + 63) & ~63;
  const int nkb = kpad / KB;
  const int my_tiles = wave < ntiles ? (ntiles - wave + NW - 1) / NW : 0;
  const int nitems = my_tiles * nkb;
  const float* arow0 = s.src + (lane & 15) * s.src_ld + 8 * (lane >> 4);
  const float* arow1 = arow0 + 16 * s.src_ld;
  const float* wbase = s.W + (size_t)(wave >> 1) * 64 * kpad + (size_t)(wave & 1) * 4 * 256;
  const unsigned lo = 4u * lane;
  const size_t tile_stride = (size_t)(NW / 2) * 64 * kpad;
  Acc32H acc;
  float4 bias4[2] = {make_float4(0.f, 0.f, 0.f, 0.f), make_float4(0.f, 0.f, 0.f, 0.f)};
  SUB_STAMP(1);
  if (CHAIN_DBG(s.dbg) & 32) return false;
  if (!preloaded) {
#pragma unroll
    for (int i = 0; i < 4; ++i) {
      w0.b[i] = ld4(wbase + (size_t)(lo + i * 256u));
      w0.b[4 + i] = ld4(wbase + (size_t)(lo + (8 + i) * 256u));
    }
    __builtin_amdgcn_sched_barrier(0);
  }
  SUB_STAMP(2);
  __builtin_amdgcn_s_waitcnt(0x0F70);
  int tt = 0, kb = 0;
  const float* wcur = wbase;
  auto run = [&](auto buf, const float* np_last) {
    constexpr int BUF = decltype(buf)::value;
    const float* np = wcur;
    int nt = tt, nk = kb;
    if (++nk == nkb) { nk = 0; ++nt; np = wbase + (size_t)nt * tile_stride; }
    else np += 16 * 256;
    const float* nload = np_last != nullptr ? np_last : np;
    if (kb == 0) {
#pragma unroll
      for (int rg = 0; rg < 2; ++rg)
#pragma unroll
        for (int jj = 0; jj < 2; ++jj) { acc.hi[rg][jj] = f32x4{0.f, 0.f, 0.f, 0.f}; acc.lo[rg][jj] = f32x4{0.f, 0.f, 0.f, 0.f}; }
      const float* bsrc = s.bias != nullptr ? s.bias : s.W;
#pragma unroll
      for (int jj = 0; jj < 2; ++jj) {
        const int c = (wave + tt * NW) * 32 + 16 * jj + 4 * (lane >> 4);
        if constexpr (NB) {
          const int cl = s.N - 1;
          bias4[jj] = make_float4(bsrc[min(c, cl)], bsrc[min(c + 1, cl)], bsrc[min(c + 2, cl)], bsrc[min(c + 3, cl)]);
        } else {
          bias4[jj] = ld4(bsrc + min(c, max(s.N - 4, 0)));
        }
      }
    }
    item32h<BUF>(acc, w0, arow0, arow1, kb * KB, nload, lo);
    SUB_STAMP(3 + tt * nkb + kb);
    if (kb == nkb - 1) {
      int tile = wave + tt * NW;
      int sidx = step_idx;
      asm volatile("" : "+s"(tile), "+s"(sidx));
      if (!(CHAIN_DBG(s.dbg) & 1)) {
        const LinSpec e = make_spec(sidx);
        if (tile * 32 + 32 <= e.N) {
          const f32x4 thi[4] = {acc.hi[0][0], acc.hi[0][1], acc.hi[1][0], acc.hi[1][1]};
          const f32x4 tlo[4] = {acc.lo[0][0], acc.lo[0][1], acc.lo[1][0], acc.lo[1][1]};
          lin_epilogue32<DROP>(e, tile * 32, thi, tlo, lane, bias4);
        } else {
          f32x4 y[4];
#pragma unroll
          for (int rg = 0; rg < 2; ++rg)
#pragma unroll
            for (int jj = 0; jj < 2; ++jj)
#pragma unroll
              for (int i = 0; i < 4; ++i)
                y[2 * rg + jj][i] = fmaf(acc.lo[rg][jj][i], 1.0f / (H_LO_SCALE * H_ACT_SCALE), acc.hi[rg][jj][i] * (1.0f / H_ACT_SCALE));
          lin_epilogue16<DROP, 2, true, 2>(e, tile * 32, y, lane, 0.0f, bias4);
        }
      }
    }
    if (nk == 0) SUB_STAMP(16 + tt);
    wcur = np; tt = nt; kb = nk;
    __builtin_amdgcn_sched_barrier(0);
  };
  using B0 = std::integral_constant<int, 0>;
  using B1 = std::integral_constant<int, 1>;
  const float* fallback = wbase;
  int it = 0;
#pragma unroll 1
  for (; it + 1 < nitems; it += 2) {
    run(B0{}, nullptr);
    const bool last = it + 2 >= nitems;
    run(B1{}, last ? (next_first != nullptr ? next_first : fallback) : nullptr);
  }
  if (it < nitems) {
    run(B0{}, fallback);
    return false;
  }
  return next_first != nullptr;
}

template <int R, bool DROP, bool SRC2, int MM, bool NB = false, typename SpecFn>
__device__ __forceinline__ bool linear_step(const LinSpec& s, WBuf& w0, bool preloaded,
                                            const float* next_first, SpecFn make_spec, int step_idx) {
  if constexpr (R == 32) return linear_step32h<DROP, NB>(s, w0, preloaded, next_first, make_spec, step_idx);
  if constexpr (R == 16 && MM == 1) return linear_step16h<DROP>(s, w0, preloaded, next_first, make_spec, step_idx);
  if constexpr (R == 16) return linear_step16<DROP, SRC2>(s, w0, preloaded, next_first, make_spec, step_idx);
  constexpr int NG = R / 4;
  const int lane = threadIdx.x & 63;
  const int wave = (__builtin_amdgcn_readfirstlane(threadIdx.x >> 6) - s.woff) & (CH_NW - 1);
  const int ntiles = (s.N + 63) >> 6;
  const int kpad = (s.K + 63) & ~63;
  const int nkb = kpad / KB;
  const int my_tiles = wave < ntiles ? (ntiles - wave + CH_NW - 1) / CH_NW : 0;
  const int nitems = my_tiles * nkb;
  const float* arow = s.src + (lane & 3) * s.src_ld + 4 * (lane >> 2);
  const float* a2row = SRC2 && s.src2 ? s.src2 + (lane & 3) * s.src2_ld + 4 * (lane >> 2) : nullptr;
  const float* wbase = s.W + 4 * lane + (size_t)wave * 64 * kpad;
  const size_t tile_stride = (size_t)CH_NW * 64 * kpad;
  Acc<NG> acc;
  float bv = 0.0f;
#ifdef TC_CHAIN_STAMPS
  constexpr bool stamp_items = true;
#else
  constexpr bool stamp_items = false;
#endif
  int tt = 0, kb = 0;
  const float* wcur = wbase;
  auto run = [&](const WBuf& wb, WBuf& nx, auto pf, const float* np_last) {
    constexpr bool PF = decltype(pf)::value;
    const float* np = wcur;
    int nt = tt, nk = kb;
    if (++nk == nkb) { nk = 0; ++nt; np = wbase + (size_t)nt * tile_stride; }
    else np += (KB / 4) * 256;
    const float* nload = np_last != nullptr ? np_last : np;
    if (stamp_items && tt == 0 && kb < 2) SUB_STAMP(20 + 5 * kb);
    if (kb == 0) {
      acc_zero<NG>(acc);
      const int col = min((wave + tt * CH_NW) * 64 + lane, s.N - 1);
      bv = ldg1((s.bias != nullptr ? s.bias : s.W) + col);
    }
    if (stamp_items && tt == 0 && kb < 2) SUB_STAMP(22 + 5 * kb);
    float4 ar[NG];
#pragma unroll
    for (int g = 0; g < NG; ++g) {
      ar[g] = *reinterpret_cast<const float4*>(arow + 4 * g * s.src_ld + kb * KB);
      if (SRC2 && a2row != nullptr)
        ar[g] = add4(ar[g], *reinterpret_cast<const float4*>(a2row + 4 * g * s.src2_ld + kb * KB));
    }
    wcompute<NG, PF>(acc, wb, ar, nx, nload);
    if (stamp_items && tt == 0 && kb < 2) SUB_STAMP(23 + 5 * kb);
    if (kb == nkb - 1) {
      int tile = wave + tt * CH_NW;
      int sidx = step_idx;
      asm volatile("" : "+s"(tile), "+s"(sidx));
      if (!(CHAIN_DBG(s.dbg) & 1)) {
        const LinSpec e = make_spec(sidx);
        lin_epilogue<NG, DROP>(e, tile, acc, lane, bv);
      }
    }
    wcur = np; tt = nt; kb = nk;
  };
  using Yes = std::integral_constant<bool, true>;
  SUB_STAMP(1);
  if (CHAIN_DBG(s.dbg) & 32) return false;
  if (!preloaded) {
    wload(w0, wbase, 16);
    __builtin_amdgcn_sched_barrier(0);
  }
  SUB_STAMP(2);
  WBuf w1;
  const float* fallback = wbase;
  int i = 0;
#pragma unroll 1
  for (; i + 1 < nitems; i += 2) {
    run(w0, w1, Yes{}, nullptr);
    __builtin_amdgcn_sched_barrier(0);
    SUB_STAMP(3 + i);
    const bool last = i + 2 >= nitems;
    run(w1, w0, Yes{}, last ? (next_first != nullptr ? next_first + 4 * lane : fallback) : nullptr);
    __builtin_amdgcn_sched_barrier(0);
    SUB_STAMP(4 + i);
  }
  if (i < nitems) {
    run(w0, w1, Yes{}, fallback);
    SUB_STAMP(3 + i);
    return false;
  }
  return next_first != nullptr;
}

template <int R, int NREC>
__device__ __forceinline__ float* buf_ptr(ChainLds<R, NREC>& S, int id) {
  switch (id) {
    case B_A: return &S.unit[1][0][0];
    case B_X: return &S.unit[0][0][0];
    case B_U1: return &S.unit[1][0][0];
    case B_U2: return &S.unit[2][0][0];
    case B_U3: return &S.unit[3][0][0];
    case B_L: return &S.l[0][0];
    default: return nullptr;
  }
}
__device__ __forceinline__ int buf_ld(int id) { return id == B_A ? LD5 : id == B_L ? LDL : LD2; }

#ifdef TC_CHAIN_STAMPS
__device__ long long g_chain_stamps[CH_NW_MAX][64];
__device__ long long g_chain_stamps2[CH_NW_MAX][64];
__device__ int g_stamp_block2 = -1;
#define STEP_STAMP()                                                                          \
  do {                                                                                        \
    if (blockIdx.x == 100 && lane == 0 && stamp_i < 64)                                       \
      g_chain_stamps[wave][stamp_i] = __builtin_amdgcn_s_memtime();                           \
    if ((int)blockIdx.x == g_stamp_block2 && lane == 0 && stamp_i < 64)                       \
      g_chain_stamps2[wave][stamp_i] = __builtin_amdgcn_s_memtime();                          \
    ++stamp_i;                                                                                \
  } while (0)
#else
#define STEP_STAMP() do {} while (0)
#endif

__device__ __forceinline__ int ufirst(int v) { return __builtin_amdgcn_readfirstlane(v); }
template <typename T>
__device__ __forceinline__ T* uptr(T* p) {
  const unsigned long long v = reinterpret_cast<unsigned long long>(p);
  const unsigned lo = __builtin_amdgcn_readfirstlane((unsigned)v);
  const unsigned hi = __builtin_amdgcn_readfirstlane((unsigned)(v >> 32));
  return reinterpret_cast<T*>(((unsigned long long)hi << 32) | lo);
}

template <typename T>
__device__ __forceinline__ T load_uniform(const T& src) {
  constexpr int NWORDS = sizeof(T) / 4;
  static_assert(sizeof(T) % 4 == 0, "record size");
  union U { T r; int w[NWORDS]; __device__ U() {} } u;
  const int* p = reinterpret_cast<const int*>(&src);
#pragma unroll
  for (int i = 0; i < NWORDS; ++i) u.w[i] = __builtin_amdgcn_readfirstlane(p[i]);
  return u.r;
}

#ifdef TC_CHAIN_STAMPS
#define START_STAMP(slot)                                                                     \
  do {                                                                                        \
    if (blockIdx.x == 100 && threadIdx.x == 0) g_chain_sub[0][(slot)] = __builtin_amdgcn_s_memtime(); \
  } while (0)
__device__ long long g_wg_span[1024][2];
#define WG_STAMP(which)                                                                       \
  do {                                                                                        \
    if (threadIdx.x == 0 && blockIdx.x < 1024) g_wg_span[blockIdx.x][(which)] = __builtin_amdgcn_s_memtime(); \
  } while (0)
__device__ unsigned g_cu_ticket[2048];
__device__ int g_wg_cu[2048][2];
#else
#define START_STAMP(slot) do {} while (0)
#define WG_STAMP(which) do {} while (0)
#endif

template <int R, int PROG, bool DROP = false, int MM = 0, bool PRE = false, bool MP = false>
__device__ __forceinline__ void chain_body(const ChainDev& k, const StepAllT<nw_of(R)>* __restrict__ recs, const int block) {
  constexpr int NW = nw_of(R), NT = NW * 64;
  constexpr bool PL = R == 32;
  static_assert((MM == 0 && R <= 16) || (MM == 1 && R >= 16 && PROG != PROG_PROLOGUE), "the f16 two-plane path exists for 16- and 32-row tiles (and is the only one at 32)");
  extern __shared__ __align__(16) unsigned char smem_raw[];
  using Lds = ChainLds<R, rec_cap(PROG)>;
  Lds& S = *reinterpret_cast<Lds*>(smem_raw);
  const int lane = threadIdx.x & 63;
  const int wave = __builtin_amdgcn_readfirstlane(threadIdx.x >> 6);
  const int m0 = block * R;
  constexpr int REC16 = rec_cap(PROG) * (int)(sizeof(StepAllT<NW>) / 16);
  constexpr int REC_TRIPS = (REC16 + NT - 1) / NT;
  int4 rec_v[REC_TRIPS];
#pragma unroll
  for (int t = 0; t < REC_TRIPS; ++t) {
    const int i = min((int)threadIdx.x + t * NT, REC16 - 1);
    rec_v[t] = reinterpret_cast<const int4*>(recs)[i];
  }
  const int M = k.M;
  if (CHAIN_DBG(k.dbg) & 64) return;
  START_STAMP(40);
  WG_STAMP(0);
#ifdef TC_CHAIN_STAMPS
  if constexpr (R == 16 && PROG == PROG_DECODER) {
    const int stg = (k.dbg >> 8) & 0xFF;
    if (stg > 0 || (k.dbg & (1 << 16))) {
      const unsigned hw = __builtin_amdgcn_s_getreg((31 << 11) | 4);
      const unsigned xcc = __builtin_amdgcn_s_getreg((3 << 11) | 20);
      const unsigned key = ((xcc & 7u) << 8) | ((hw >> 8) & 0xFFu);
      unsigned tk = 0;
      if (threadIdx.x == 0) {
        tk = atomicAdd(&g_cu_ticket[key], 1u);
        if (blockIdx.x < 2048) { g_wg_cu[blockIdx.x][0] = (int)key; g_wg_cu[blockIdx.x][1] = (int)tk; }
      }
      tk = (unsigned)__builtin_amdgcn_readfirstlane((int)tk);
      if (wave == 0 && tk == 1u) {
#pragma unroll 1
        for (int i = 0; i < stg; ++i) __builtin_amdgcn_s_sleep(64);
      }
    }
  }
#endif
  const int total = k.total;
  constexpr int EARLY_MAX = 3, EARLY_RW = (R + NW - 1) / NW;
  const int early_n = k.early_n;
  {
    float4 early_v[EARLY_MAX][EARLY_RW];
#pragma unroll
    for (int j = 0; j < EARLY_MAX; ++j) {
      if (j < early_n) {
        const float* gsrc = recs[j].r.gd;
        const int ld = recs[j].r.gld, mod = recs[j].r.gmod;
#pragma unroll
        for (int ri = 0; ri < EARLY_RW; ++ri) {
          int grow = min(m0 + wave + ri * NW, M - 1);
          if (mod > 0) grow = grow % mod;
          early_v[j][ri] = TC_ONCE_LD(gsrc + (size_t)grow * ld + 4 * lane);
        }
      }
    }
    START_STAMP(41);
#pragma unroll
    for (int j = 0; j < EARLY_MAX; ++j) {
      if (j < early_n) {
        float* dst = reinterpret_cast<float*>(smem_raw) + recs[j].e.dst_off;
#pragma unroll
        for (int ri = 0; ri < EARLY_RW; ++ri) {
          const int row = wave + ri * NW;
          if (row < R) act_st4<PL>(dst + row * LD2, 4 * lane, early_v[j][ri]);
        }
      }
    }
  }
#pragma unroll
  for (int t = 0; t < REC_TRIPS; ++t) {
    const int i = threadIdx.x + t * NT;
    if (i < REC16) reinterpret_cast<int4*>(&S.recs[0])[i] = rec_v[t];
  }
  START_STAMP(43);

  if (prog_is_radar(PROG)) {
    auto row_of = [&](int row) {
      const int pos = min(m0 + row, M - 1);
      return k.row_perm != nullptr ? k.row_perm[pos] : pos;
    };
    if (threadIdx.x < R) S.rowg[threadIdx.x] = row_of(threadIdx.x);
// ... 19 lines not shown
      }
    }
  }
  if constexpr (PROG == PROG_RADAR_BWD) {
    for (int i = threadIdx.x; i < R * LD2; i += NT) (&S.unit[0][0][0])[i] = 0.0f;
    if (threadIdx.x < R * 12) (&S.box[0][0])[threadIdx.x] = 0.0f;
    if (threadIdx.x < R) S.gate[threadIdx.x] = 0;
  }
  __syncthreads();

  START_STAMP(46);
#ifdef TC_CHAIN_STAMPS
  int stamp_i = 0;
  STEP_STAMP();
#endif

  auto do_ln = [&](const StepRes& r) {
    constexpr int NR = R / NW;
    const float* a = buf_ptr(S, r.src); const int lda = buf_ld(r.src);
    const float* c = buf_ptr(S, r.src2); const int ldc = buf_ld(r.src2);
    const bool xp = (r.flags & F_LN_XP) != 0;
    const float* dd = xp ? nullptr : buf_ptr(S, r.res);
    float* dst2 = xp ? buf_ptr(S, r.res) : nullptr;
    float* dst = buf_ptr(S, r.dst);
    float* gdst = r.gd;
    float4 gg, bb;
    if (CHAIN_DBG(k.dbg) & (1 << 17)) {
      gg = make_float4(1.f, 1.f, 1.f, 1.f); bb = make_float4(0.f, 0.f, 0.f, 0.f);
    } else {
      gg = ld4(r.p0 + 4 * lane); bb = ld4(r.p1 + 4 * lane);
    }
    float4 v[NR], pos4[NR];
#pragma unroll
    for (int i = 0; i < NR; ++i) {
      const int row = wave + NW * i;
      pos4[i] = make_float4(0.f, 0.f, 0.f, 0.f);
      if (xp && !(CHAIN_DBG(k.dbg) & (1 << 18))) {
        int prow = min(m0 + row, M - 1);
        if (k.g_mod[G_POS] > 0) prow = prow % k.g_mod[G_POS];
        pos4[i] = ld4(k.g[G_POS] + (size_t)prow * k.g_ld[G_POS] + 4 * lane);
      }
      v[i] = act_ld4<PL>(a + row * lda, 4 * lane);
    }
    if (c != nullptr) {
      const float4 g2 = ld4(r.p2 + 4 * lane), b2 = ld4(r.p3 + 4 * lane);
      float4 cv[NR];
#pragma unroll
      for (int i = 0; i < NR; ++i) cv[i] = act_ld4<PL>(c + (wave + NW * i) * ldc, 4 * lane);
      ln_rows<NR>(cv, g2, b2);
#pragma unroll
      for (int i = 0; i < NR; ++i) v[i] = add4(v[i], relu4(cv[i]));
    }
    ln_rows<NR>(v, gg, bb);
#pragma unroll
    for (int i = 0; i < NR; ++i) {
      const int row = wave + NW * i;
      if (r.flags & F_LN_RELU) v[i] = relu4(v[i]);
      if constexpr (PROG == PROG_RADAR_ENC_TRAIN) {
        if (r.gt != nullptr && m0 + row < M) st4(r.gt + (size_t)(m0 + row) * 256 + 4 * lane, v[i]);
      }
      if (dd != nullptr) v[i] = add4(v[i], act_ld4<PL>(dd + row * LD2, 4 * lane));
      act_st4<PL>(dst + row * LD2, 4 * lane, v[i]);
      if (xp) act_st4<PL>(dst2 + row * LD2, 4 * lane, add4(v[i], pos4[i]));
      if (gdst != nullptr && m0 + row < M) st4(gdst + (size_t)(m0 + row) * 256 + 4 * lane, v[i]);
    }
  };
  auto lin_spec = [&](const StepRes& r) {
    LinSpec s;
    s.K = r.K; s.N = r.N;
    s.W = r.p0; s.bias = r.p1;
    const float* lbase = reinterpret_cast<const float*>(smem_raw);
    s.src = lbase + r.src_off; s.src_ld = buf_ld(r.src);
    s.src2 = r.src2_off >= 0 ? lbase + r.src2_off : nullptr; s.src2_ld = buf_ld(r.src2);
    s.dst = nullptr; s.dst_ld = 0; s.res = nullptr; s.res_ld = 0; s.gate = nullptr;
    s.act = 0; s.scale = 1.0f; s.scale_cols = 0;
    s.gdst = nullptr; s.gdst_ld = 0; s.gt = nullptr; s.gt_ld = 0; s.gt_rpb = 1;
    s.m0 = m0; s.M = M;
    s.woff = (r.flags & F_WAVE1) ? 1 : 0;
    s.dbg = k.dbg;
    s.sub_on = 0;
    s.drop_site = 0; s.drop_seed = 0; s.drop_thr = 0; s.drop_scale = 1.0f; s.drop_stride = 0; s.drop_q = 0;
    s.rowg = nullptr; s.gpre = 0; s.cmask = nullptr; s.cscale = 1.0f;
    s.dst_pl = 0; s.res_pl = 0; s.range_flag = nullptr;
    return s;
  };
  auto epi_spec = [&](int j) {
    const EpiRec e = load_uniform<EpiRec>(S.recs[j].e);
    float* base = reinterpret_cast<float*>(smem_raw);
    LinSpec s;
    s.K = 0; s.N = e.N; s.W = nullptr;
    s.bias = e.has_bias ? base : nullptr;
    s.src = nullptr; s.src_ld = 0; s.src2 = nullptr; s.src2_ld = 0;
    s.dst = e.dst_off >= 0 ? base + e.dst_off : nullptr; s.dst_ld = e.dst_ld;
    s.res = e.res_off >= 0 ? base + e.res_off : nullptr; s.res_ld = e.res_ld;
    s.gate = (e.flags & F_GATE) ? &S.gate[0] : nullptr;
    s.act = e.act;
    s.scale = (e.flags & F_SCALEQ) ? k.qscale : 1.0f; s.scale_cols = (e.flags & F_SCALEQ) ? 256 : 0;
    s.gdst = e.gd; s.gdst_ld = e.gld;
    s.gt = (e.flags & F_CMASK) ? nullptr : e.gt; s.gt_ld = k.qpad; s.gt_rpb = k.Q;
    s.cmask = (e.flags & F_CMASK) ? e.gt : nullptr;
    s.cscale = (e.flags & F_CMASK_SCALE) ? k.rdrop.scale : 1.0f;
    s.m0 = m0; s.M = M;
    s.woff = e.woff;
    s.dbg = 0;
    s.sub_on = 0;
    s.drop_site = 0; s.drop_seed = 0; s.drop_thr = 0; s.drop_scale = 1.0f; s.drop_stride = 0; s.drop_q = 0;
    s.rowg = (prog_is_radar(PROG) && k.row_perm != nullptr) ? &S.rowg[0] : nullptr;
    s.gpre = (e.flags & F_GPRE) ? 1 : 0;
    s.dst_pl = PL && e.dst_ld != LDL; s.res_pl = PL && e.res_ld != LDL;
    s.range_flag = MM == 1 ? k.range_status : nullptr;
    if (DROP) {
      if constexpr (PROG == PROG_RADAR_TRAIN) {
        s.drop_site = e.drop_site; s.drop_seed = k.rdrop.seed; s.drop_thr = k.rdrop.thr; s.drop_scale = k.rdrop.scale;
      } else {
        s.drop_site = e.drop_site; s.drop_seed = k.drop.seed; s.drop_thr = k.drop.thr; s.drop_scale = k.drop.scale;
        s.drop_stride = k.drop.seed_stride; s.drop_q = (int)k.drop.rows_per_sample;
      }
    }
    return s;
  };

  auto tile_has_hit = [&]() {
    int any = 0;
#pragma unroll
    for (int i = 0; i < R; ++i) any |= S.gate[i];
    return __builtin_amdgcn_readfirstlane(any) > 0;
  };

#ifdef TC_CHAIN_DUMP
  auto dump_step = [&](int step, int dst_id) {
    if constexpr (PROG == PROG_RADAR) {
      __syncthreads();
      float* out = g_chain_dump;
      const float* src = buf_ptr(S, dst_id);
      if (out != nullptr && src != nullptr && dst_id != B_L && (long long)(step + 1) * M * 256 <= g_chain_dump_floats) {
        const int ld = buf_ld(dst_id);
        for (int row = wave; row < R; row += NW)
          if (m0 + row < M)
            st4(out + ((size_t)step * M + S.rowg[row]) * 256 + 4 * lane, *reinterpret_cast<const float4*>(src + row * ld + 4 * lane));
      }
      __syncthreads();
    }
  };
#define DUMP_STEP(step, dst) dump_step((step), (dst))
#else
#define DUMP_STEP(step, dst) do {} while (0)
#endif
  int idx = (CHAIN_DBG(k.dbg) & 16) ? total : early_n;
#ifdef TC_CHAIN_STAMPS
  for (int j = 0; j < 2 * early_n; ++j) STEP_STAMP();
#endif
#pragma unroll 1
  while (idx < total) {
    const int kind = ufirst(S.recs[idx].r.kind);
    if (kind == K_LINEAR || kind == K_LN || kind == K_NOP) {
      WBuf w0;
      int pre_idx = -1;
#ifdef TC_CHAIN_STAMPS
      int ln_rep = 0;
#endif
#pragma unroll 1
      for (;;) {
        const StepRes r = load_uniform<StepRes>(S.recs[idx].r);
        const int kd = r.kind;
        bool skip = false;
        if constexpr (PROG == PROG_RADAR) {
          if (kd == K_LINEAR && (r.flags & F_IFHIT)) skip = !tile_has_hit();
        }
        if (skip) {
          if (r.res != B_NONE && r.dst != B_NONE) {
            const float* rs = buf_ptr(S, r.res); const int rld = buf_ld(r.res);
            float* dd = buf_ptr(S, r.dst);
            for (int row = wave; row < R; row += NW)
              *reinterpret_cast<float4*>(dd + row * LD2 + 4 * lane) = *reinterpret_cast<const float4*>(rs + row * rld + 4 * lane);
          }
        } else if (kd == K_LINEAR) {
          LinSpec s = lin_spec(r);
#ifdef TC_CHAIN_STAMPS
          s.sub_on = (r.si == g_sub_step && r.rep == 0);
          SUB_STAMP(0);
#endif
          if (((wave - s.woff) & (NW - 1)) < (R == 32 ? (s.N + 31) >> 5 : (s.N + 63) >> 6)) {
            const PreRec pr = load_uniform<PreRec>(S.recs[idx].p[wave]);
            const bool have = linear_step<R, DROP, PROG == PROG_PROLOGUE, MM, MP>(s, w0, pre_idx == idx, pr.first, epi_spec, idx);
            pre_idx = have ? pr.nidx : -1;
          }
        } else if (kd == K_LN) {
          if (!(CHAIN_DBG(k.dbg) & 4)) do_ln(r);
#ifdef TC_CHAIN_STAMPS
          if (ln_rep < ((k.dbg >> 19) & 3)) { ++ln_rep; continue; }
          ln_rep = 0;
#endif
        } else if (kd != K_NOP) {
          break;
        }
        STEP_STAMP();
        if (r.sync && !(CHAIN_DBG(k.dbg) & 2)) __syncthreads();
        STEP_STAMP();
        DUMP_STEP(idx, r.dst);
        if (++idx >= total) break;
      }
      continue;
    }
    const StepRes r = load_uniform<StepRes>(S.recs[idx].r);
    const int rep = r.rep;
    switch (kind) {
      case K_LOAD: { if constexpr (PROG == PROG_DECODER || PROG == PROG_PROLOGUE || PROG == PROG_RADAR_ENC_B) {
        constexpr int MAXL = 3, RW = (R + NW - 1) / NW;
        int n = 1;
        while (n < MAXL && idx + n < total && ufirst(S.recs[idx + n].r.kind) == K_LOAD) ++n;
        float4 v[MAXL][RW];
        float* dsts[MAXL];
        int any_sync = 0;
#pragma unroll
        for (int j = 0; j < MAXL; ++j) {
          if (j < n) {
            const StepRes rj = load_uniform<StepRes>(S.recs[idx + j].r);
            const float* gsrc = rj.gd;
            const int ld = rj.gld, mod = rj.gmod;
            dsts[j] = buf_ptr(S, rj.dst);
            any_sync |= rj.sync;
#pragma unroll
            for (int ri = 0; ri < RW; ++ri) {
              int grow = min(m0 + wave + ri * NW, M - 1);
              if (mod > 0) grow = grow % mod;
              v[j][ri] = TC_ONCE_LD(gsrc + (size_t)grow * ld + 4 * lane);
            }
          }
        }
#pragma unroll
        for (int j = 0; j < MAXL; ++j) {
          if (j < n) {
#pragma unroll
            for (int ri = 0; ri < RW; ++ri) {
              const int row = wave + ri * NW;
              if (row < R) act_st4<PL>(dsts[j] + row * LD2, 4 * lane, v[j][ri]);
            }
          }
        }
        for (int j = 0; j < n; ++j) { STEP_STAMP(); STEP_STAMP(); }
        if (any_sync) __syncthreads();
        idx += n;
        continue;
      }
      } break;
      case K_TOKENS: { if constexpr (prog_is_enc_full(PROG) || PROG == PROG_RADAR_ENC_A) {
        if constexpr (PL) {
          for (int i = threadIdx.x; i < R * 16; i += NT) {
            const int row = i >> 4, c4 = 4 * (i & 15);
            const int grow = min(m0 + row, M - 1);
            const float* tk = k.tokens + (size_t)grow * k.RI;
            act_st4<PL>(&S.unit[1][0][0] + row * LD5, c4,
                        make_float4(c4 < k.RI ? tk[c4] : 0.0f, c4 + 1 < k.RI ? tk[c4 + 1] : 0.0f, c4 + 2 < k.RI ? tk[c4 + 2] : 0.0f,
                                    c4 + 3 < k.RI ? tk[c4 + 3] : 0.0f));
          }
        } else {
        for (int i = threadIdx.x; i < R * 64; i += NT) {
          const int row = i >> 6, c = i & 63;
          const int grow = min(m0 + row, M - 1);
          (&S.unit[1][0][0])[row * LD5 + c] = c < k.RI ? k.tokens[(size_t)grow * k.RI + c] : 0.0f;
        }
        }
      } break;
      } break;
      case K_POSENC: { if constexpr (PROG == PROG_DECODER || prog_is_enc_full(PROG) || PROG == PROG_RADAR_ENC_A) {
        float* dst = buf_ptr(S, r.dst);
        const bool skip0 = (r.flags & F_NOT_W0) != 0;
// ... 445 lines not shown
            const float4 dO = *reinterpret_cast<const float4*>(dao + row * LD2 + 4 * lane);
            dq = radar_attn_bwd_row(cxy[0], cxy[1], bx[3], bx[6], bx[7], k.rmin[layer], k.rmax[layer], q4,
                                    k.tokens + (size_t)b * k.T * k.RI, k.RI, uptr(r.p2) + (size_t)b * k.T * 512,
                                    const_cast<float*>(uptr(r.p3)) + (size_t)b * k.T * 512, 512, k.T, k.pad_mult, dO, o4,
                                    dk, grow, lane,
                                    k.detp != nullptr ? det_shadow_of(*k.detp, uptr(r.p3) + (size_t)b * k.T * 512) : nullptr);
            dq.x *= k.qscale; dq.y *= k.qscale; dq.z *= k.qscale; dq.w *= k.qscale;
          }
          *reinterpret_cast<float4*>(dqb + row * LD2 + 4 * lane) = dq;
          if (r.gd != nullptr && m0 + row < M) st4(r.gd + (size_t)grow * 256 + 4 * lane, dq);
        }
      } break;
      } break;
      case K_BOXADD: { if constexpr (prog_is_radar(PROG)) {
        const int row = threadIdx.x >> 4, j = threadIdx.x & 15;
        if (row < R && j < k.code) {
          const int c = j == 0 ? 0 : j == 1 ? 1 : j == 4 ? 2 : -1;
          float bx = S.l[row][j];
          if (c >= 0) { bx += S.cen[row][c]; S.cen[row][c] = bx; }
          S.box[row][j] = bx;
          if (m0 + row < M) k.all_box[((size_t)rep * M + S.rowg[row]) * k.code + j] = bx;
        }
      } break;
      } break;
      case K_BOXSIG: { if constexpr (PROG == PROG_DECODER_HEADS) {
        const int row = threadIdx.x >> 4, j = threadIdx.x & 15;
        if (row < R && m0 + row < M && j < k.code) {
          const int grow = m0 + row;
          float val = S.l[row][j];
          const int c = j == 0 ? 0 : j == 1 ? 1 : j == 4 ? 2 : -1;
          if (c >= 0) {
            const float n = sigmoidf_(val + inverse_sigmoidf_(ldg1(r.p0 + (size_t)grow * 3 + c)));
            const float* pc = k.cam.pc;
            val = n * (pc[3 + c] - pc[c]) + pc[c];
          }
          stg1(r.gd + (size_t)grow * k.code + j, val);
        }
      } break;
      } break;
      default: break;
    }
    STEP_STAMP();
    if (r.sync) __syncthreads();
    STEP_STAMP();
    DUMP_STEP(idx, r.dst);
    ++idx;
  }
  WG_STAMP(1);
}

template <int R, int PROG, bool DROP = false, int MM = 0, bool PRE = false, bool MP = false>
__global__ __launch_bounds__(nw_of(R) * 64, 2) void chain_kernel(ChainDev k, Recs<rec_cap(PROG), nw_of(R)> recs) {
  chain_body<R, PROG, DROP, MM, PRE, MP>(k, recs.s, blockIdx.x);
}

template <int RA, int RB, int PROGB, int MM = 0, bool PRE = false, bool MP = false>
__global__ __launch_bounds__(nw_of(RA) * 64, 2) void chain_dual_kernel(ChainDev ka, ChainDev kb, int na,
                                                           Recs<rec_cap(PROG_DECODER), nw_of(RA)> ra,
                                                           Recs<rec_cap(PROGB), nw_of(RB)> rb) {
  static_assert(nw_of(RA) == nw_of(RB), "both programs of a launch run with the same workgroup size");
  if ((int)blockIdx.x < na) chain_body<RA, PROG_DECODER, false, MM, PRE, MP>(ka, ra.s, blockIdx.x);
  else chain_body<RB, PROGB, false, MM>(kb, rb.s, (int)blockIdx.x - na);
}

template <int R, int PROG>
int lds_off(int id) {
  using Lds = ChainLds<R, rec_cap(PROG)>;
  const int unit0 = (int)(offsetof(Lds, unit) / 4), ustride = R * LD2;
  switch (id) {
    case B_A: return unit0 + ustride;
    case B_X: return unit0;
    case B_U1: return unit0 + ustride;
    case B_U2: return unit0 + 2 * ustride;
    case B_U3: return unit0 + 3 * ustride;
    case B_L: return (int)(offsetof(Lds, l) / 4);
    default: return -1;
  }
}
template <int R, int PROG>
constexpr size_t chain_lds_bytes() { return sizeof(ChainLds<R, rec_cap(PROG)>); }
static_assert(chain_lds_bytes<16, PROG_RADAR>() <= 80 * 1024 && chain_lds_bytes<32, PROG_RADAR>() <= 160 * 1024, "radar programs: LDS per workgroup");
inline int buf_ld_h(int id) { return id == B_A ? LD5 : id == B_L ? LDL : LD2; }

template <int R, int PROG, int MM = 0>
void resolve_program(ChainK& k, StepAllT<nw_of(R)>* out) {
  constexpr int NW = nw_of(R);
  const StepDesc* table = prog_table(PROG);
  int nsteps = table_steps(PROG);
  if (PROG == PROG_DECODER && k.l0_seq != 0) {
    table = k.l0_seq == 1 ? PROG_DECODER_L0_T : PROG_DECODER_L0GEN_T;
    nsteps = (int)((k.l0_seq == 1 ? sizeof(PROG_DECODER_L0_T) : sizeof(PROG_DECODER_L0GEN_T)) / sizeof(StepDesc)) - 1;
  }
  if (prog_is_enc_full(PROG) || PROG == PROG_RADAR_ENC_A || PROG == PROG_RADAR_ENC_B)
    while (nsteps > 0 && table[nsteps - 1].kind == K_LINEAR && table[nsteps - 1].wp >= 7 + k.nlayers) --nsteps;
  const int nrep = (prog_is_radar(PROG) || PROG == PROG_RADAR_BWD) ? k.nlayers : 1;
  const int total = nsteps * nrep;
  memset(out, 0, sizeof(StepAllT<NW>) * rec_cap(PROG));
  for (int idx = 0; idx < total; ++idx) {
    const int rep = idx / nsteps, si = idx - rep * nsteps;
    const int layer = PROG == PROG_RADAR_BWD ? k.nlayers - 1 - rep : rep;
    const int pair0 = (prog_is_radar(PROG) || PROG == PROG_RADAR_BWD) ? layer * RADAR_PAIRS : 0;
    const StepDesc d = table[si];
    StepRes& r = out[idx].r;
    r.K = d.K; r.N = d.N;
    r.kind = d.kind; r.src = d.src; r.src2 = d.src2; r.dst = d.dst; r.res = d.res; r.act = d.act;
    r.flags = d.flags; r.sync = d.sync; r.rep = (short)rep; r.si = (short)si;
    if ((d.flags & F_SKIP_NONEXT) && !k.has_next) r.kind = K_NOP;
    if (PROG == PROG_DECODER && !k.refine &&
        (d.kind == K_REFUPD || ((d.kind == K_LINEAR || d.kind == K_NARROW) && d.wp >= 13 && d.wp <= 15)))
      r.kind = K_NOP;
    if (PROG == PROG_RADAR && k.last_cls_only && rep + 1 < nrep && d.wp >= 6 && d.wp <= 10 &&
        (d.kind == K_LINEAR || d.kind == K_LN || d.kind == K_NARROW))
      r.kind = K_NOP;
    if (d.gsel != G_NONE) { r.gd = k.g[d.gsel]; r.gld = k.g_ld[d.gsel]; r.gmod = k.g_mod[d.gsel]; }
    if (d.gtsel != G_NONE) r.gt = k.g[d.gtsel];
    bool taped = false;
    if (PROG == PROG_RADAR_TRAIN) {
      if (d.flags & F_SCALEQ) r.flags = (short)(r.flags & ~F_SCALEQ);
      r.flags = (short)(r.flags & ~F_IFHIT);
      if (d.kind == K_LINEAR && d.wp == 4) r.flags = (short)(r.flags | F_GPRE);
      const short ts = RADAR_TAPE[si];
      if (ts != T_NONE && r.gd == nullptr) { r.gd = k.tape[ts] + (size_t)rep * k.tape_stride; r.gld = 256; taped = true; }
    }
    if (PROG == PROG_RADAR_BWD) {
      if ((d.flags & F_NOT_LAYER0) && layer == 0) r.kind = K_NOP;
      const short ds = BWD_STORE[si], ts = BWD_TAPE[si], ts2 = BWD_TAPE2[si];
      if (ds != D_NONE && k.dy[ds] != nullptr) { r.gd = k.dy[ds] + (size_t)layer * k.dy_stride; taped = true; }
      const float* t1 = ts != T_NONE ? k.tape[ts] + (size_t)layer * k.tape_stride : nullptr;
      const float* t2 = ts2 != T_NONE ? k.tape[ts2] + (size_t)layer * k.tape_stride : nullptr;
      if (d.kind == K_LINEAR && (d.flags & F_CMASK)) r.gt = const_cast<float*>(t1);
      if (d.kind == K_LN_BWD) {
        const tc_linear n = k.pairs[pair0 + d.wp], gn = k.gpairs[pair0 + d.wp];
        r.p0 = n.w; r.p1 = t1; r.p2 = t2; r.gt = const_cast<float*>(gn.w); r.p3 = gn.b;
      }
      if (d.kind == K_LOADG) {
        r.N = d.N == N_CODE ? k.code : k.ncls;
        r.p0 = (d.N == N_CODE ? k.d_box : k.d_cls) + (size_t)layer * k.M * r.N;
      }
      if (d.kind == K_MASKCOPY) r.K = d.K;
      if (d.kind == K_ATTN_BWD) {
        r.p0 = k.tape[T_QP] + (size_t)layer * k.tape_stride; r.p1 = k.tape[T_AO] + (size_t)layer * k.tape_stride;
        r.p2 = k.g[G_KV0 + layer]; r.p3 = k.dkv[layer];
      }
    }
    if (PROG == PROG_RADAR_ENC_TRAIN) {
      const short ts = ENC_TAPE[si], ts2 = ENC_TAPE2[si];
      if (ts != T_NONE && r.gd == nullptr) { r.gd = k.tape[ts]; r.gld = 256; taped = true; }
      if (ts2 != T_NONE) r.gt = k.tape[ts2];
    }
    if (PROG == PROG_DECODER && d.N == N_LOGITS && generic_xattn(k)) r.dst = B_U3;
    if (PROG == PROG_DECODER_HEADS) {
      if (d.kind == K_NARROW && 16 * d.act >= (d.N == N_CODE ? k.code : k.ncls)) r.kind = K_NOP;
      if (d.kind == K_BOXSIG) { r.p0 = k.ref_in; r.gd = k.box_m; r.gld = k.code; }
    }
    if (d.kind == K_LINEAR) {
      const tc_linear pr = k.pairs[pair0 + d.wp];
      r.K = d.K == 36 ? k.RI : d.K == N_CODE ? k.code : d.K == N_CLS ? k.ncls : d.K;
      r.N = d.N == N_LOGITS ? k.nlogits : d.N == N_CODE ? k.code : d.N == N_CLS ? k.ncls : d.N;
      const int woff = (d.flags & F_WOFF) ? 512 : 0;
      r.p0 = pr.w + (size_t)woff * ((r.K + 63) & ~63);
      if (R >= 16) r.p0 += (MM == 1 ? 2 : 1) * k.w16_delta;
      r.p1 = pr.b ? pr.b + woff : nullptr;
      if (PROG == PROG_RADAR_BWD) r.p1 = nullptr;
      if (d.gsel == G_CLS) r.gd += (size_t)rep * k.M * k.ncls;
      if (taped) r.gld = r.N;
    } else if (d.kind == K_NARROW) {
      const tc_linear pr = k.pairs[pair0 + d.wp];
      r.N = d.N == N_CODE ? k.code : d.N == N_CLS ? k.ncls : d.N;
      r.p0 = pr.w; r.p1 = pr.b;
      if (d.gsel == G_CLS) r.gd += (size_t)rep * k.M * k.ncls;
      if (taped) r.gld = r.N;
    } else if (d.kind == K_LN || d.kind == K_POSENC) {
      const tc_linear n = k.pairs[pair0 + d.wp];
      r.p0 = n.w; r.p1 = n.b;
      if (d.kind == K_POSENC || d.src2 != B_NONE) {
        const tc_linear n2 = k.pairs[pair0 + d.wp2];
        r.p2 = n2.w; r.p3 = n2.b;
      }
    }
    r.src_off = lds_off<R, PROG>(r.src); r.src2_off = lds_off<R, PROG>(r.src2);
    EpiRec& e = out[idx].e;
    e.gd = r.gd; e.gt = r.gt; e.gld = r.gld; e.act = r.act; e.flags = r.flags; e.N = r.N;
    e.has_bias = r.p1 != nullptr; e.woff = (r.flags & F_WAVE1) ? 1 : 0;
    e.drop_site = 0;
    if (PROG == PROG_DECODER && k.drop.thr != 0 && d.kind == K_LINEAR) {
      const int off = d.wp == 1 ? 1 : d.wp == 4 ? 2 : d.wp == 10 ? 3 : d.wp == 11 ? 4 : 0;
      if (off) e.drop_site = (int)k.drop.site + off + 1;
    }
    if (PROG == PROG_RADAR_TRAIN && d.kind == K_LINEAR) {
      const int off = d.wp == 1 ? 1 : d.wp == 3 ? 2 : d.wp == 4 ? 3 : 0;
      if (off) e.drop_site = 4 * rep + off + 1;
    }
    e.dst_off = lds_off<R, PROG>(r.dst); e.dst_ld = buf_ld_h(r.dst);
    e.res_off = lds_off<R, PROG>(r.res); e.res_ld = buf_ld_h(r.res);
  }
  for (int idx = 0; idx < total; ++idx) {
    for (int w = 0; w < NW; ++w) {
      PreRec& pr = out[idx].p[w];
      pr.first = nullptr; pr.nidx = -1;
      for (int j = idx + 1; j < total; ++j) {
        const StepRes& n = out[j].r;
        if (n.kind == K_LN || n.kind == K_NOP) continue;
        if (n.kind != K_LINEAR) break;
        const int vw = (w - ((n.flags & F_WAVE1) ? 1 : 0)) & (NW - 1);
        const size_t kpad = (size_t)((n.K + 63) & ~63);
        if (R == 32) {
          if (vw >= ((n.N + 31) >> 5)) continue;
          pr.nidx = j;
          pr.first = n.p0 + (size_t)(vw >> 1) * 64 * kpad + (size_t)(vw & 1) * 4 * 256;
        } else {
          if (vw >= ((n.N + 63) >> 6)) continue;
          pr.nidx = j;
          pr.first = n.p0 + (size_t)vw * 64 * kpad;
        }
        break;
      }
    }
  }
  k.total = total;
  int early = 0;
  while (early < 3 && early < total && out[early].r.kind == K_LOAD) ++early;
  k.early_n = early;
}

template <class Kernel>
int allow_lds(DeviceOnce& once, Kernel kernel, size_t lds) {
  if (const int dev = once.need(); dev >= 0) {
    hipError_t e = hipFuncSetAttribute(reinterpret_cast<const void*>(kernel), hipFuncAttributeMaxDynamicSharedMemorySize, (int)lds);
    if (e != hipSuccess) { set_error("chain: hipFuncSetAttribute: %s", hipGetErrorString(e)); return (int)e; }
    once.done(dev);
  }
  return 0;
}

int need_packed16(int R, size_t w16_delta, const char* what, const char* packer = "tc_head_pack_weights") {
  TC_REQUIRE(R < 16 || w16_delta != 0, "%s: 16- / 32-row tiles need weights from a %s view (packed16_delta is 0)", what, packer);
  return 0;
}

tc_linear ln_pair(const tc_lnorm& n) { return tc_linear{n.g, n.b}; }

template <int RA, int RB, int PROGB, int MM = 0, bool PRE = false, bool MP = false>
int launch_dual_r(const ChainK& ka_, const ChainK& kb_, hipStream_t s, const char* what) {
  constexpr size_t lds = chain_lds_bytes<RA, PROG_DECODER>() > chain_lds_bytes<RB, PROGB>() ? chain_lds_bytes<RA, PROG_DECODER>() : chain_lds_bytes<RB, PROGB>();
  static DeviceOnce once;
  if (const int rc = allow_lds(once, chain_dual_kernel<RA, RB, PROGB, MM, PRE, MP>, lds)) return rc;
  ChainK ka = ka_, kb = kb_;
  if (const int rc = need_packed16(RA, ka.w16_delta, what) | need_packed16(RB, kb.w16_delta, what)) return rc;
  Recs<rec_cap(PROG_DECODER), nw_of(RA)> ra;
  Recs<rec_cap(PROGB), nw_of(RB)> rb;
  resolve_program<RA, PROG_DECODER, MM>(ka, ra.s);
  resolve_program<RB, PROGB, MM>(kb, rb.s);
  const int na = (ka.M + RA - 1) / RA, nb = (kb.M + RB - 1) / RB;
  hipLaunchKernelGGL((chain_dual_kernel<RA, RB, PROGB, MM, PRE, MP>), dim3(na + nb), dim3(nw_of(RA) * 64), lds, s,
                     static_cast<const ChainDev&>(ka), static_cast<const ChainDev&>(kb), na, ra, rb);
  return check_launch(what);
}

template <int R, int PROG, bool DROP = false, int MM = 0, bool PRE = false, bool MP = false>
int launch_r(const ChainK& k_, hipStream_t s, const char* what) {
  constexpr size_t lds = chain_lds_bytes<R, PROG>();
  static DeviceOnce once;
  if (const int rc = allow_lds(once, chain_kernel<R, PROG, DROP, MM, PRE, MP>, lds)) return rc;
  ChainK k = k_;
  if (const int rc = need_packed16(R, k.w16_delta, what)) return rc;
  Recs<rec_cap(PROG), nw_of(R)> recs;
  resolve_program<R, PROG, MM>(k, recs.s);
  hipLaunchKernelGGL((chain_kernel<R, PROG, DROP, MM, PRE, MP>), dim3((k.M + R - 1) / R), dim3(nw_of(R) * 64), lds, s,
                     static_cast<const ChainDev&>(k), recs);
  return check_launch(what);
}

#ifdef TC_CHAIN_STAMPS
static int g_dbg_override = -1;
#endif
void init_k(ChainK& k) {
  memset(&k, 0, sizeof(k));
#ifdef TC_CHAIN_STAMPS
  static const int dbg = [] { const char* e = getenv("TRANSCAR_CHAIN_DBG"); return e ? atoi(e) : 0; }();
  k.dbg = g_dbg_override >= 0 ? g_dbg_override : dbg;
#endif
}

template <class F>
int with_variant(int v, F&& f) {
  switch (v) {
    case TV_4: return f(std::integral_constant<int, TV_4>{});
    case TV_8: return f(std::integral_constant<int, TV_8>{});
    case TV_16_F32: return f(std::integral_constant<int, TV_16_F32>{});
    case TV_16_F16X2: return f(std::integral_constant<int, TV_16_F16X2>{});
    case TV_32_F16X2: return f(std::integral_constant<int, TV_32_F16X2>{});
    default: return -1;
  }
}

template <int PROG, bool MP = false>
int launch_rows(const ChainK& k, hipStream_t s, const char* what) {
  return with_variant(tile_variant(k.M, k.tile_rows, k.matrix_path, what), [&](auto V) {
    constexpr int R = variant_rows(V), MM = variant_mm(V);
    if constexpr (PROG == PROG_DECODER && MM == 1) { if (k.pre != nullptr) return launch_r<R, PROG, false, MM, true, MP>(k, s, what); }
    return launch_r<R, PROG, false, MM, false, MP>(k, s, what);
  });
}

constexpr int drop_variant(int v) { return v == TV_16_F32 ? TV_8 : v; }

template <bool MP>
int launch_decoder(const ChainK& k, hipStream_t s, const char* what) {
  if (k.drop.thr == 0) return launch_rows<PROG_DECODER, MP>(k, s, what);
  TC_REQUIRE((unsigned long long)(k.drop.rows_per_sample ? k.drop.rows_per_sample : k.M) * 512ull < (1ull << 32),
             "decoder_chain: dropout index space");
  return with_variant(tile_variant(k.M, k.tile_rows, k.matrix_path, what), [&](auto V) {
    constexpr int W = drop_variant(V);
    return launch_r<variant_rows(W), PROG_DECODER, true, variant_mm(W), false, MP>(k, s, what);
  });
}

constexpr int HEADS_STEPS = table_steps(PROG_DECODER_HEADS);
template <int NW> struct HeadsRecs { StepAllT<NW> s[TC_MAX_LAYERS * HEADS_STEPS]; };
template <int R, int MM>
__global__ __launch_bounds__(nw_of(R) * 64, 2) void chain_heads_kernel(ChainDev k, int tiles, HeadsRecs<nw_of(R)> recs) {
  const int level = (int)blockIdx.x / tiles;
  chain_body<R, PROG_DECODER_HEADS, false, MM>(k, recs.s + level * HEADS_STEPS, (int)blockIdx.x - level * tiles);
}

ChainK heads_level_k(const DecoderHeadsArgs& a, int l) {
  ChainK k;
  init_k(k);
  k.program = PROG_DECODER_HEADS; k.M = a.M; k.Q = a.M; k.code = a.code; k.ncls = a.ncls; k.has_next = 1;
  k.w16_delta = a.w16_delta; k.matrix_path = a.matrix_path; k.range_status = a.range_status;
  const tc_cls_branch& c = a.cls[l]; const tc_reg_branch& g = a.reg[l];
  k.pairs[0] = c.l0; k.pairs[1] = ln_pair(c.n1); k.pairs[2] = c.l3; k.pairs[3] = ln_pair(c.n4);
  k.pairs[4] = c.l6; k.pairs[5] = g.l0; k.pairs[6] = g.l2; k.pairs[7] = g.l4;
  k.g[G_HS] = const_cast<float*>(a.hs) + (size_t)l * a.M * 256; k.g_ld[G_HS] = 256;
  k.g[G_CLS] = a.all_cls + (size_t)l * a.M * a.ncls; k.g_ld[G_CLS] = a.ncls;
  k.ref_in = l == 0 ? a.init_ref : a.inter_refs + (size_t)(l - 1) * a.M * 3;
  k.box_m = a.all_box + (size_t)l * a.M * a.code;
  for (int i = 0; i < 6; ++i) k.cam.pc[i] = a.pc[i];
  return k;
}

template <int R, int MM>
int launch_heads_r(const DecoderHeadsArgs& a, hipStream_t s) {
  const char* what = "chain(decoder heads)";
  constexpr size_t lds = chain_lds_bytes<R, PROG_DECODER_HEADS>();
  static DeviceOnce once;
  if (const int rc = allow_lds(once, chain_heads_kernel<R, MM>, lds)) return rc;
  if (const int rc = need_packed16(R, a.w16_delta, what, "tc_decoder_heads_pack")) return rc;
  HeadsRecs<nw_of(R)> recs;
  memset(&recs, 0, sizeof(recs));
// ... 343 lines not shown
}
__device__ __forceinline__ float sc_value(unsigned long long h, int kind) {
  const float u = (float)(h >> 40) * (1.0f / 16777216.0f) * 2.0f - 1.0f;
  const int e = (int)((h >> 8) & 63) - 44;
  switch (kind & 15) {
    case 0: return 0.0f;
    case 1: return -0.0f;
    case 2: return __builtin_bit_cast(float, (unsigned)(h & 0x007FFFFFu));
    case 3: return ldexpf(u, -20);
    case 4: return u * 70000.0f * 64.0f;
    case 5: return (h & 1) ? INFINITY : -INFINITY;
    case 6: return __builtin_bit_cast(float, 0x7FC00000u | (unsigned)(h & 0xFFFFu));
    default: return ldexpf(u, e);
  }
}
__device__ __forceinline__ bool sc_differ(float a, float b) {
  if (a != a && b != b) return false;
  return __builtin_bit_cast(unsigned, a) != __builtin_bit_cast(unsigned, b);
}
__global__ __launch_bounds__(256) void rowops_selfcheck_kernel(unsigned long long seed, unsigned long long* mismatches) {
  const int lane = threadIdx.x & 63, wave = threadIdx.x >> 6;
  unsigned long long bad0 = 0, bad1 = 0, bad2 = 0;
  const unsigned long long base = sc_mix(seed + 0x9E3779B97F4A7C15ull * (unsigned long long)(blockIdx.x * 4 + wave + 1));
  {
    float4 v[4], w1[4];
    const unsigned long long hg = sc_mix(base + 77 + (unsigned long long)lane);
    const float4 gg = make_float4(sc_value(hg, 8), sc_value(sc_mix(hg + 1), 8), sc_value(sc_mix(hg + 2), 8), sc_value(sc_mix(hg + 3), 8));
    const float4 bb = make_float4(sc_value(sc_mix(hg + 4), 8), sc_value(sc_mix(hg + 5), 8), sc_value(sc_mix(hg + 6), 8), sc_value(sc_mix(hg + 7), 8));
#pragma unroll
    for (int i = 0; i < 4; ++i) {
      const unsigned long long hr = sc_mix(base + 1000ull * (unsigned long long)(i + 1));
      const float mag = ldexpf(1.0f, (int)(hr & 31) - 16), off = (hr & 32) ? mag * (float)((hr >> 6) & 1023) : 0.0f;
      const int flavour = (int)((hr >> 20) & 7);
      float x[4];
#pragma unroll
      for (int c = 0; c < 4; ++c) {
        const unsigned long long he = sc_mix(hr + 16ull * (unsigned long long)lane + (unsigned long long)c);
        const float u = (float)(he >> 40) * (1.0f / 16777216.0f) * 2.0f - 1.0f;
        x[c] = flavour == 0 ? off + mag : flavour == 1 ? off + ((lane == 17 && c == 2) ? mag * 1000.0f : mag * 1e-3f * u) : off + mag * u;
      }
      v[i] = make_float4(x[0], x[1], x[2], x[3]);
      w1[i] = v[i];
    }
    ln_rows<4>(v, gg, bb);
#pragma unroll
    for (int i = 0; i < 4; ++i) {
      float4 one[1] = {w1[i]};
      ln_rows<1>(one, gg, bb);
      bad0 += sc_differ(one[0].x, v[i].x) + sc_differ(one[0].y, v[i].y) + sc_differ(one[0].z, v[i].z) + sc_differ(one[0].w, v[i].w);
    }
  }
  __shared__ float lds[4][64][8];
  for (int it = 0; it < 64; ++it) {
    const unsigned long long h0 = sc_mix(base + 31ull * (unsigned long long)(it * 64 + lane) + 5);
    const unsigned long long h1 = sc_mix(h0 + 1);
    const float t0 = sc_value(h0, (int)(h0 >> 4)), t1 = sc_value(h1, (int)(h1 >> 4));
    unsigned hi, lo;
    split_t2(t0, t1, hi, lo);
    const unsigned rh = pk_h2(t0, t1);
    const f16x2 hv = __builtin_bit_cast(f16x2, rh);
    const f16x2 rl = {(_Float16)((t0 - (float)hv[0]) * H_LO_SCALE), (_Float16)((t1 - (float)hv[1]) * H_LO_SCALE)};
    const f16x2 gh = __builtin_bit_cast(f16x2, hi), gl = __builtin_bit_cast(f16x2, lo);
    bad1 += sc_differ((float)gh[0], (float)hv[0]) + sc_differ((float)gh[1], (float)hv[1]) +
            sc_differ((float)gl[0], (float)rl[0]) + sc_differ((float)gl[1], (float)rl[1]);
    const unsigned long long h2 = sc_mix(h0 + 2), h3 = sc_mix(h0 + 3);
    const float4 x4 = make_float4(t0, t1, sc_value(h2, (int)(h2 >> 4)), sc_value(h3, (int)(h3 >> 4)));
    float* row = &lds[wave][lane][0];
    act_st4<true>(row, 0, x4);
    const float4 g4 = act_ld4<true>(row, 0);
    const char* pp = reinterpret_cast<const char*>(row);
    const uint2 ph = *reinterpret_cast<const uint2*>(pp), pl = *reinterpret_cast<const uint2*>(pp + 16);
    const f16x2 a0 = __builtin_bit_cast(f16x2, ph.x), a1 = __builtin_bit_cast(f16x2, ph.y);
    const f16x2 b0 = __builtin_bit_cast(f16x2, pl.x), b1 = __builtin_bit_cast(f16x2, pl.y);
    constexpr float UH = 1.0f / H_ACT_SCALE, UL = 1.0f / (H_ACT_SCALE * H_LO_SCALE);
    bad2 += sc_differ(g4.x, fmaf((float)b0[0], UL, (float)a0[0] * UH)) + sc_differ(g4.y, fmaf((float)b0[1], UL, (float)a0[1] * UH)) +
            sc_differ(g4.z, fmaf((float)b1[0], UL, (float)a1[0] * UH)) + sc_differ(g4.w, fmaf((float)b1[1], UL, (float)a1[1] * UH));
  }
  if (bad0) atomicAdd(mismatches + 0, bad0);
  if (bad1) atomicAdd(mismatches + 1, bad1);
  if (bad2) atomicAdd(mismatches + 2, bad2);
}
}

int launch_rowops_selfcheck(int n_blocks, unsigned long long seed, unsigned long long* mismatches, hipStream_t s) {
  TC_REQUIRE(n_blocks > 0 && mismatches != nullptr, "rowops_selfcheck: bad arguments");
  hipLaunchKernelGGL(rowops_selfcheck_kernel, dim3(n_blocks), dim3(256), 0, s, seed, mismatches);
  return check_launch("rowops_selfcheck");
}

}
```

### transcar_amd/csrc/head.hip

```cpp
#include <math.h>
#include <stdarg.h>
#include <stdlib.h>
#include <string.h>

#include "kernels.hpp"

namespace tc {

static thread_local char g_err[512] = "";

void set_error(const char* fmt, ...) {
  va_list ap;
  va_start(ap, fmt);
  vsnprintf(g_err, sizeof(g_err), fmt, ap);
  va_end(ap);
}

int check_launch(const char* what) {
  hipError_t e = hipGetLastError();
  if (e != hipSuccess) {
    set_error("%s: %s", what, hipGetErrorString(e));
    return (int)e;
  }
  return 0;
// ... 603 lines not shown
  if (tile_variant(0, opt.chain_tile_rows, opt.matrix_path, "the row chains") < 0) {
    char why[200];
    snprintf(why, sizeof(why), "%s", g_err);
    TC_REQUIRE(false, "options.chain_tile_rows=%d, options.matrix_path=%d: %s", opt.chain_tile_rows, opt.matrix_path, why);
  }
  TC_REQUIRE(opt.decoder_dropout_p >= 0.0f && opt.decoder_dropout_p < 1.0f, "options.decoder_dropout_p=%g",
             (double)opt.decoder_dropout_p);
  TC_REQUIRE(opt.phase >= 0 && opt.phase <= 2, "options.phase=%d (0 whole forward, 1 before the radar tokens, 2 the rest)",
             opt.phase);
  TC_REQUIRE(opt.phase == 0 || !opt.unfused, "options.phase=%d needs the fused path", opt.phase);
  TC_REQUIRE(opt.cam_pregather == 0 || opt.cam_pregather == 1, "options.cam_pregather=%d (0 off, 1 on)", opt.cam_pregather);
  TC_REQUIRE(opt.cam_pregather == 0 || opt.cam_pregather_ws != nullptr, "options.cam_pregather needs cam_pregather_ws");
  return 0;
}

int tc_radar_fusion_fwd(const tc_head_weights* packed_view, const float* hs_last, const float* ref_last,
                        const float* prev_box, const float* radar_tokens, int B, int T, int pad_mult,
                        int first_layer, int num_layers, float* all_cls_scores, float* all_bbox_preds,
                        int* hit_counts, const tc_head_options* options, void* workspace,
                        size_t workspace_bytes, tc_stream_t stream) {
  const tc_head_weights* w = packed_view;
  TC_TRY(check_dims(w));
  TC_REQUIRE(w->l0_attn_out != nullptr, "radar_fusion: packed_view was not produced by tc_head_pack_weights");
  TC_REQUIRE(first_layer >= 0 && num_layers >= 1 && first_layer + num_layers <= w->num_radar_layers,
             "radar_fusion: layers [%d, %d) of %d", first_layer, first_layer + num_layers, w->num_radar_layers);
  TC_REQUIRE(hs_last && prev_box && radar_tokens && all_cls_scores && all_bbox_preds && (first_layer > 0 || ref_last),
             "radar_fusion: null argument");
  TC_REQUIRE(B >= 1 && T >= 1 && pad_mult >= 1, "radar_fusion: B=%d T=%d pad_mult=%d", B, T, pad_mult);
  tc_head_options opt;
  TC_TRY(read_options(options, opt));
  HeadWs h;
  const size_t need = head_ws_layout(w, B, T, workspace, workspace_bytes, &h);
  TC_REQUIRE(need <= workspace_bytes, "workspace too small: need %zu, have %zu", need, workspace_bytes);
  hipStream_t s = as_stream(stream);
  const int Q = w->num_query, C = w->embed_dims, rows = B * Q, rt = B * T;
  const int code = w->code_size, ncls = w->num_classes;
  RadarEncodeArgs re;
  re.tokens = radar_tokens; re.RI = w->radar_in_dims; re.M = rt;
  re.rpe = w->radar_position_encoder; re.f0 = w->radar_feat0; re.f2 = w->radar_feat2;
  re.f4 = w->radar_feat4; re.nlayers = w->num_radar_layers;
  for (int r = 0; r < TC_MAX_RADAR_LAYERS; ++r) {
    const tc_mha& m = w->radar[r].attn;
    re.kvproj[r] = tc_linear{m.in_proj.w ? m.in_proj.w + (size_t)C * C : nullptr,
                             m.in_proj.b ? m.in_proj.b + C : nullptr};
    re.kv[r] = h.kv3[r];
  }
  re.radar_feat = h.radar_feat;
  re.w16_delta = w->packed16_delta; re.matrix_path = opt.matrix_path;
  if (!opt.reuse_radar_kv) TC_TRY(launch_radar_encode(re, s));
  RadarChainArgs rc;
  rc.qf = hs_last; rc.ref_last = ref_last; rc.box_m = prev_box; rc.tokens = radar_tokens;
  rc.RI = w->radar_in_dims;
  for (int r = 0; r < num_layers; ++r) { rc.kv[r] = h.kv3[first_layer + r]; rc.w[r] = w->radar[first_layer + r]; }
  rc.nlayers = num_layers; rc.Q = Q; rc.T = T; rc.pad_mult = pad_mult; rc.code = code; rc.ncls = ncls;
  rc.M = rows; rc.qscale = 1.0f / sqrtf((float)(C / TC_RADAR_HEADS));
  for (int i = 0; i < 6; ++i) rc.pc[i] = w->pc_range[i];
  rc.all_cls = all_cls_scores + (size_t)first_layer * rows * ncls;
  rc.all_box = all_bbox_preds + (size_t)first_layer * rows * code;
  rc.hits = h.hits; rc.tile_rows = opt.chain_tile_rows; rc.last_cls_only = opt.last_level_cls_only; rc.matrix_path = opt.matrix_path;
  rc.range_status = opt.range_status;
  rc.cen_from_box = first_layer > 0;
  if (opt.radar_row_order == 2 || (opt.radar_row_order == 0 && rows > 1024)) {
    TC_TRY(launch_radar_compact(ref_last, prev_box, code, rc.cen_from_box, w->pc_range, radar_tokens, w->radar_in_dims,
                                B, Q, T, w->radar[first_layer].radius_min, w->radar[first_layer].radius_max,
                                h.hitflag, h.perm, s));
    rc.row_perm = h.perm;
  }
  TC_TRY(launch_radar_chain(rc, s));
  if (hit_counts != nullptr)
    TC_HIP(hipMemcpyAsync(hit_counts + (size_t)first_layer * rows, h.hits, (size_t)num_layers * rows * 4,
                          hipMemcpyDeviceToDevice, s));
  return 0;
}

int tc_radar_gate_selfcheck(int n_radii, unsigned long long seed, unsigned long long* mismatches,
                            tc_stream_t stream) {
  return launch_gate_selfcheck(n_radii, seed, mismatches, as_stream(stream));
}

int tc_rowops_selfcheck(int n_blocks, unsigned long long seed, unsigned long long* mismatches, tc_stream_t stream) {
  return launch_rowops_selfcheck(n_blocks, seed, mismatches, as_stream(stream));
}

size_t tc_box_decode_workspace_bytes(int B, int Q, int num_classes) {
  return box_decode_ws_bytes(B, Q, num_classes);
}

int tc_box_decode_topk(const float* cls_scores, const float* bbox_preds, int B, int Q,
                       int num_classes, int code_size, int max_num, const float* post_center_range,
                       float* boxes, float* scores, int* labels, unsigned char* valid,
                       void* workspace, size_t workspace_bytes, tc_stream_t stream) {
  return launch_box_decode(cls_scores, bbox_preds, B, Q, num_classes, code_size, max_num,
                           post_center_range, boxes, scores, labels, valid, workspace,
                           workspace_bytes, as_stream(stream));
}

int tc_box_decode_kept(const float* cls_scores, const float* bbox_preds, int B, int Q, int num_classes, int code_size,
                       int max_num, const float* post_center_range, float score_threshold, int use_threshold,
                       int z_shift, float* kept_boxes, float* kept_scores, long long* kept_labels, int* kept_count,
                       tc_stream_t stream) {
  BoxDecodeKept k{kept_boxes, kept_scores, kept_labels, kept_count, score_threshold, use_threshold, z_shift};
  return launch_box_decode(cls_scores, bbox_preds, B, Q, num_classes, code_size, max_num, post_center_range,
                           nullptr, nullptr, nullptr, nullptr, nullptr, 0, as_stream(stream), &k);
}

int tc_box_decode_topk_path(const float* cls_scores, const float* bbox_preds, int B, int Q,
                            int num_classes, int code_size, int max_num, const float* post_center_range,
                            float* boxes, float* scores, int* labels, unsigned char* valid,
                            void* workspace, size_t workspace_bytes, tc_stream_t stream, int path) {
  return launch_box_decode(cls_scores, bbox_preds, B, Q, num_classes, code_size, max_num,
                           post_center_range, boxes, scores, labels, valid, workspace,
                           workspace_bytes, as_stream(stream), nullptr, path);
}

int tc_box_decode_kept_path(const float* cls_scores, const float* bbox_preds, int B, int Q, int num_classes, int code_size,
                            int max_num, const float* post_center_range, float score_threshold, int use_threshold,
                            int z_shift, float* kept_boxes, float* kept_scores, long long* kept_labels, int* kept_count,
                            tc_stream_t stream, int path) {
  BoxDecodeKept k{kept_boxes, kept_scores, kept_labels, kept_count, score_threshold, use_threshold, z_shift};
  return launch_box_decode(cls_scores, bbox_preds, B, Q, num_classes, code_size, max_num, post_center_range,
                           nullptr, nullptr, nullptr, nullptr, nullptr, 0, as_stream(stream), &k, path);
}

size_t tc_head_packed_bytes(const tc_head_weights* w) {
  if (check_dims(w) != 0) return 0;
  bool refine;
  if (decoder_refines(w, &refine) != 0) return 0;
  tc_head_weights view = *w;
  PackItem items[MAX_PACK_ITEMS];
  const int n = collect_pack_items(w, &view, items);
  size_t total = 0;
  for (int i = 0; i < n; ++i)
    if (!items[i].narrow && !items[i].absent) total += 3 * arena_slice(packed_floats(items[i].N, items[i].K), 4);
  const size_t Q = w->num_query, C = w->embed_dims;
  total += arena_slice(Q * 3, 4) + arena_slice(Q * C, 4) + l0_scratch_bytes(w);
  return total;
}

int tc_head_pack_weights(const tc_head_weights* w, void* packed, size_t packed_bytes,
                         tc_head_weights* packed_view, tc_stream_t stream) {
  TC_TRY(check_dims(w));
  bool refine;
  TC_TRY(decoder_refines(w, &refine));
  TC_REQUIRE(packed != nullptr && packed_view != nullptr, "pack_weights: null output");
  TC_REQUIRE(packed_bytes >= tc_head_packed_bytes(w), "pack_weights: buffer too small");
  *packed_view = *w;
  PackItem items[MAX_PACK_ITEMS];
  const int n = collect_pack_items(w, packed_view, items);
  Arena a(packed, packed_bytes);
  size_t region_a = 0;
  for (int i = 0; i < n; ++i)
    if (!items[i].narrow && !items[i].absent) region_a += arena_slice(packed_floats(items[i].N, items[i].K), 4);
  const size_t delta = region_a / sizeof(float);
  for (int i = 0; i < n; ++i) {
    if (items[i].absent) { *items[i].slot = nullptr; continue; }
    TC_REQUIRE(items[i].src != nullptr, "pack_weights: weight %d is null", i);
    if (items[i].narrow) continue;
    float* dst = a.take<float>(packed_floats(items[i].N, items[i].K));
    TC_TRY(launch_pack_linear(items[i].src, items[i].N, items[i].K, dst, dst + delta, dst + 2 * delta, as_stream(stream)));
    *items[i].slot = dst;
  }
  for (int rgn = 0; rgn < 2; ++rgn)
    for (int i = 0; i < n; ++i)
      if (!items[i].narrow && !items[i].absent) a.take<float>(packed_floats(items[i].N, items[i].K));
  packed_view->packed16_delta = delta;
  for (int l = 0; l < TC_MAX_LAYERS; ++l) packed_view->layers[l].packed16_delta = delta;
// ... 446 lines not shown
```

### transcar_amd/csrc/kernels.hpp

```cpp
#pragma once
#include "common.hpp"
#include "../../include/transcar_hip.h"

namespace tc {

struct GemmArgs {
  const float* X = nullptr;  int ldx = 0;
  const float* X2 = nullptr; int x2_cols = 0;
  const float* W = nullptr;  int ldw = 0;
  const float* bias = nullptr;
  const float* R = nullptr;  int ldr = 0;
  const int* rowgate = nullptr;
  float* Y = nullptr;        int ldy = 0;
  float* Yt = nullptr;
  int t_col0 = 0, t_ld = 0, t_rows_per_batch = 1;
  int M = 0, K = 0, N = 0;
  int act = 0;
  float scale = 1.0f; int scale_cols = 0;
};
int launch_gemm(const GemmArgs& a, hipStream_t s);

struct LnArgs {
  const float* a = nullptr;
  const float* b = nullptr;
// ... 69 lines not shown
  const float* pre = nullptr; const int* premask = nullptr;
  const float* l0_consts = nullptr;
};
int launch_decoder_chain(const DecoderChainArgs& a, hipStream_t s);
constexpr int TC_L0_VARIANTS = TV_COUNT;
size_t decoder_l0_const_floats(int Q);
int launch_decoder_l0_consts(const DecoderChainArgs& a, int variant, float* consts, hipStream_t s);

struct RadarEncodeArgs {
  const float* tokens; int RI, M;
  tc_pos_encoder rpe; tc_linear f0, f2, f4;
  int nlayers; tc_linear kvproj[TC_MAX_RADAR_LAYERS]; float* kv[TC_MAX_RADAR_LAYERS];
  float* radar_feat;
  size_t w16_delta = 0;
  float* const* tape = nullptr;
  int matrix_path = 0;
  int* range_status = nullptr;
};
int launch_radar_encode(const RadarEncodeArgs& a, hipStream_t s);
int launch_decoder_chain_with_encoders(const DecoderChainArgs& d, const RadarEncodeArgs& e, int part,
                                       hipStream_t s);

struct RadarChainArgs {
  const float* qf; const float* ref_last; const float* box_m;
  const float* tokens; int RI;
  const float* kv[TC_MAX_RADAR_LAYERS];
  tc_radar_layer w[TC_MAX_RADAR_LAYERS];
  int nlayers, Q, T, pad_mult, code, ncls, M;
  float qscale; float pc[6];
  float* all_cls; float* all_box; int* hits;
  int tile_rows = 0;
  int matrix_path = 0;
  int last_cls_only = 0;
  int cen_from_box = 0;
  const int* row_perm = nullptr;
  float* const* tape = nullptr; size_t tape_stride = 0, hits_stride = 0;
  DropK drop = DropK{0, 0, 1.0f, 0, 1500, 0, 0, 0};
  int* range_status = nullptr;
};
enum DySlot { DY_DBOX = 0, DY_DT1, DY_DT0, DY_DC2, DY_DC0, DY_DFF, DY_DH, DY_DPROJ, DY_DQP, DY_DCLS, DY_COUNT };
struct RadarBwdChainArgs {
  tc_radar_layer wT[TC_MAX_RADAR_LAYERS];
  tc_radar_layer w[TC_MAX_RADAR_LAYERS];
  tc_radar_layer grads[TC_MAX_RADAR_LAYERS];
  const float* kv[TC_MAX_RADAR_LAYERS]; float* dkv[TC_MAX_RADAR_LAYERS];
  const float* cxy[TC_MAX_RADAR_LAYERS]; int ld_c[TC_MAX_RADAR_LAYERS]; const float* box[TC_MAX_RADAR_LAYERS];
  float* const* tape; size_t tape_stride, hits_stride; const int* hits;
  float* const* dy; size_t dy_stride;
  const float* d_cls; const float* d_box;
  const float* loss_vals = nullptr;
  float* loss_out = nullptr;
  const float* tokens; int RI, T, pad_mult;
  int nlayers, Q, M, code, ncls;
  float qscale;
  DropK drop;
  int tile_rows = 0;
  const DetAcc* det_device = nullptr;
};
int launch_radar_chain_bwd(const RadarBwdChainArgs& a, hipStream_t s);
enum TapeSlot { TS_QP = 0, TS_AO, TS_X1, TS_X2, TS_H, TS_SUM, TS_X3, TS_C0, TS_C1, TS_C2, TS_C3, TS_T0, TS_T1, TS_TREG,
                TS_U0, TS_U1, TS_U2, TS_POS, TS_F0, TS_F1, TS_F2, TS_MEM, TS_COUNT };
int launch_radar_chain(const RadarChainArgs& a, hipStream_t s);

struct DecoderHeadsArgs {
  int levels, M;
  tc_cls_branch cls[TC_MAX_LAYERS]; tc_reg_branch reg[TC_MAX_LAYERS];
  size_t w16_delta = 0;
  const float* hs;
  const float* init_ref;
  const float* inter_refs;
  float* all_cls; float* all_box;
  int ncls, code; float pc[6];
  int tile_rows = 0, matrix_path = 0;
  int* range_status = nullptr;
};
int launch_decoder_heads(const DecoderHeadsArgs& a, hipStream_t s);

int launch_radar_compact(const float* ref_last, const float* box, int code, int cen_from_box,
                         const float* pc6_host, const float* tokens, int RI, int B, int Q, int T,
                         float rmin, float rmax, int* flags, int* perm, hipStream_t s);

int launch_gate_selfcheck(int n_radii, unsigned long long seed, unsigned long long* mismatches, hipStream_t s);
int launch_rowops_selfcheck(int n_blocks, unsigned long long seed, unsigned long long* mismatches, hipStream_t s);

inline bool heads_ok(int num_heads) { return num_heads == 4 || num_heads == 8 || num_heads == 16; }
int launch_self_attn_core(const float* q, const float* k, int ld, const float* vt, int ldt,
                          float* out, int ldo, int B, int Q, int H, int D, hipStream_t s,
                          const DropK* drop = nullptr);
struct PreGatherArgs {
  CamSampleArgs cam; int M, ref_mod; float* out; int* mask;
};
int launch_self_attn_core_x(const float* q, const float* k, int ld, const float* vt, int ldt, float* out, int ldo,
                            int B, int Q, int H, int D, hipStream_t s, const DropK* drop = nullptr,
                            const PreGatherArgs* pregather = nullptr);

struct RadarAttnArgs {
  const float* qproj; int ldq;
  const float* kv; int ldkv;
  const float* centre_xy; int ld_c;
  const float* box; int code;
  const float* radar_xy; int ld_xy;
  int B, Q, T, C, H, pad_mult;
  float rmin, rmax;
  float* attn_out;
  int* hit_counts;
  float qscale = 1.0f;
  DropK drop = DropK{0, 0, 1.0f, 0, 1500, 0, 0, 0};
};
int launch_radar_attn(const RadarAttnArgs& a, hipStream_t s);
int launch_dropout(const float* x, const float* res, const int* gate, int rows, int cols, const DropK& d,
                   float* out, hipStream_t s);

int launch_linear_bwd_data(const float* dy, const float* relu_out, const int* row_gate,
                           const float* w, const float* in_relu_mask, float* dx, int M, int K,
                           int N, float alpha, int accumulate, hipStream_t s);
int launch_linear_bwd_weight(const float* x, const float* dy, const float* relu_out,
                             const int* row_gate, float* dw, float* db, int M, int K, int N,
                             float alpha, hipStream_t s);
struct WeightJob { const float* x; const float* dy; float* dw; float* db; int M, K, N; const float* relu = nullptr;
                   int ldx = 0;  };
int launch_linear_bwd_weight_group(const WeightJob* jobs, int n, hipStream_t s);
DetAcc& current_det();
DetAcc*& current_det_device();
struct DetScope {
  DetAcc saved; DetAcc* saved_dev;
  DetScope(const DetAcc& d, DetAcc* dev) : saved(current_det()), saved_dev(current_det_device()) { current_det() = d; current_det_device() = dev; }
  ~DetScope() { current_det() = saved; current_det_device() = saved_dev; }
  DetScope(const DetScope&) = delete;
  DetScope& operator=(const DetScope&) = delete;
};
int launch_det_flush(const DetAcc& d, int range, hipStream_t s);
int launch_det_store(const DetAcc& d, DetAcc* dst, hipStream_t s);
int launch_ln256_bwd(const float* a, const float* b, const float* gamma, const float* dy,
                     const float* relu_out, float* dz, float* dgamma, float* dbeta, int M,
                     hipStream_t s);
int launch_radar_attn_bwd(const RadarAttnArgs& a, float qscale, const float* d_attn, float* dq,
                          float* dkv, hipStream_t s);
int launch_box_ref_bwd(const float* d_box, int code, float* d_prev, int M, hipStream_t s);
int launch_sqnorm(const float* g, size_t n, float* out, hipStream_t s);
int launch_adamw(float* p, const float* g, float* m, float* v, size_t n, float lr, float b1,
                 float b2, float eps, float wd, int step, float grad_scale, float max_norm,
                 const float* sqnorm, hipStream_t s);

size_t packed_floats(int N, int K);
int launch_pack_linear(const float* W, int N, int K, float* P, float* P16, float* PH, hipStream_t s);
struct PackJob { const float* W; float* P; float* P16; int N, K; int transpose = 0, ldw = 0; float* PH = nullptr; };
int launch_pack_group(const PackJob* jobs, int n, hipStream_t s);

int launch_nchw_to_nhwc(const float* src, float* dst, int n_img, int C, int H, int W, hipStream_t s);
int launch_nchw_to_nhwc_levels(const float* const* src, float* const* dst, int num_levels, int n_img,
                               int C, const int* H, const int* W, hipStream_t s);

int launch_radar_ingest(const double* raw, const double* times, const int* chan_start_host, int num_chan,
                        const double* radar_rot_host, const double* lidar_rot_host,
                        const double* point_range_host, float* tokens, int T, int* count, hipStream_t s);
int launch_radar_ingest_batch(const double* raw, const double* times, const tc_radar_frame_desc* desc, int P, int cap,
                              float* tokens, int T, int* count, hipStream_t s);

struct BoxDecodeKept {
  float* boxes; float* scores; long long* labels; int* count;
  float score_threshold; int use_threshold;
  int z_shift;
};
int launch_box_decode(const float* cls, const float* box, int B, int Q, int ncls, int code,
                      int max_num, const float* pcr6_host, float* boxes, float* scores, int* labels,
                      unsigned char* valid, void* ws, size_t ws_bytes, hipStream_t s, const BoxDecodeKept* kept = nullptr,
// ... 5 lines not shown
```

Baseline: 10340.

## Fuse LayerNorm into 32-row linear-step epilogues for the radar chain program

Measured after the change: 10410, median of 5. No clear change (+0.7%).

```diff
diff --git a/include/transcar_hip.h b/include/transcar_hip.h
--- a/include/transcar_hip.h
+++ b/include/transcar_hip.h
@@ -233,6 +233,9 @@
                             tc_stream_t stream);
 
 int tc_rowops_selfcheck(int n_blocks, unsigned long long seed, unsigned long long* mismatches, tc_stream_t stream);
+
+int tc_ln_epilogue_selfcheck(const float* x, const float* gamma, const float* beta, float* y, int n_tiles, int fused,
+                             tc_stream_t stream);
 
 size_t tc_box_decode_workspace_bytes(int B, int Q, int num_classes);
 int tc_box_decode_topk(const float* cls_scores ,
diff --git a/transcar_amd/_lib.py b/transcar_amd/_lib.py
--- a/transcar_amd/_lib.py
+++ b/transcar_amd/_lib.py
@@ -233,6 +233,7 @@
     'tc_radar_xattn_workspace_bytes': (_sz, [_i, _i, _i, _i]),
     'tc_radar_gate_selfcheck': (_i, [_i, C.c_ulonglong, _vp, _vp]),
     'tc_rowops_selfcheck': (_i, [_i, C.c_ulonglong, _vp, _vp]),
+    'tc_ln_epilogue_selfcheck': (_i, [_vp, _vp, _vp, _vp, _i, _i, _vp]),
     'tc_radar_gated_xattn_fwd': (_i, [_P(tc_mha), _vp, _vp, _vp, _i, _vp, _vp,
                                       _i, _i, _i, _i, _i, _i, _f, _f, _vp,
                                       _vp, _vp, _sz, _vp]),
diff --git a/transcar_amd/csrc/chain.hip b/transcar_amd/csrc/chain.hip
--- a/transcar_amd/csrc/chain.hip
+++ b/transcar_amd/csrc/chain.hip
@@ -45,7 +45,7 @@
   int gld, act, flags, N;
   int has_bias, woff;
   int drop_site;
-  int pad1;
+  int aux_off;
 };
 struct PreRec { const float* first; int nidx; int pad; };
 template <int NW> struct StepAllT { StepRes r; EpiRec e; PreRec p[NW]; };
@@ -55,6 +55,8 @@
 
 constexpr int HM_WORDS = 8;
 static_assert(HM_WORDS * 8 <= LDL * 4 && (LDL * 4) % 8 == 0, "hit masks live in a row of the logit buffer");
+template <int R> struct LnPart {};
+template <> struct LnPart<32> { float p[32][8][2]; };
 template <int R, int NREC>
 struct ChainLds {
   StepAllT<nw_of(R)> recs[NREC];
@@ -64,6 +66,7 @@
   float cen[R][4];
   int gate[R];
   int rowg[R];
+  [[no_unique_address]] LnPart<R> lnpart;
 };
 static_assert(LD5 * 1 <= 2 * LD2, "the 512-wide tile must fit two units");
 
@@ -103,6 +106,10 @@
   F_CARRY = 4096,
   F_NOT_LAYER0 = 8192,
   F_PRESYNC = 16384
+};
+enum EpiLn : int {
+  E_LN = 1 << 16,
+  E_LN_RES2 = 1 << 17
 };
 enum GSel : short {
   G_NONE = -1, G_HS = 0, G_QK, G_VT, G_INITREF, G_ATTN_O, G_XIN, G_POS, G_CLS, G_KV0, G_KV1, G_KV2,
@@ -257,6 +264,10 @@
 enum Program : int { PROG_PROLOGUE = 0, PROG_DECODER, PROG_RADAR_ENC, PROG_RADAR, PROG_RADAR_ENC_A, PROG_RADAR_ENC_B,
                      PROG_RADAR_TRAIN, PROG_RADAR_ENC_TRAIN, PROG_RADAR_BWD, PROG_DECODER_HEADS };
 constexpr bool prog_is_radar(int p) { return p == PROG_RADAR || p == PROG_RADAR_TRAIN; }
+constexpr bool LN32_DECODER = false;
+constexpr bool fuses_ln32(int R, int prog, int MM, bool drop, bool mp) {
+  return R == 32 && MM == 1 && !drop && !mp && ((LN32_DECODER && prog == PROG_DECODER) || prog == PROG_RADAR);
+}
 constexpr bool prog_is_enc_full(int p) { return p == PROG_RADAR_ENC || p == PROG_RADAR_ENC_TRAIN; }
 enum TSel : short { T_NONE = -1, T_QP = 0, T_AO, T_X1, T_X2, T_H, T_FF, T_X3, T_C0, T_C1, T_C2, T_C3, T_T0, T_T1, T_TREG,
                     E_U0, E_U1, E_U2, E_POS, E_F0, E_F1, E_F2, E_MEM, T_COUNT };
@@ -360,6 +371,11 @@
   const float* cmask; float cscale;
   int dst_pl, res_pl;
   int* range_flag;
+  const float* ln_g; const float* ln_b;
+  int ln_flags;
+  float* ln_aux;
+  float* ln_part;
+  const float* pos; int pos_ld, pos_mod;
 };
 
 constexpr int KB = 64;
@@ -820,8 +836,69 @@
   }
 }
 
+__device__ __forceinline__ float sum_lanes_16_32(float x) {
+  float a = x, b = x;
+  asm volatile("s_nop 1\n\tv_permlane32_swap_b32 %0, %1\n\ts_nop 1\n\tv_add_f32 %0, %0, %1\n\tv_mov_b32 %1, %0\n\ts_nop 1\n\t"
+               "v_permlane16_swap_b32 %0, %1\n\ts_nop 1\n\tv_add_f32 %0, %0, %1"
+               : "+v"(a), "+v"(b));
+  return a;
+}
+
+__device__ __forceinline__ void ln_stage32(float (&t)[4][4], const float4 (&gs)[2], const float4 (&bs)[2], float* part, int tile,
+                                           int c, int g) {
+  float mw[2], qw[2];
+#pragma unroll
+  for (int rg = 0; rg < 2; ++rg) {
+    const float* a = t[2 * rg]; const float* b = t[2 * rg + 1];
+    mw[rg] = sum_lanes_16_32(((a[0] + a[1]) + (a[2] + a[3])) + ((b[0] + b[1]) + (b[2] + b[3]))) * (1.0f / 32.0f);
+  }
+#pragma unroll
+  for (int rg = 0; rg < 2; ++rg) {
+    float q = 0.0f;
+#pragma unroll
+    for (int jj = 0; jj < 2; ++jj)
+#pragma unroll
+      for (int i = 0; i < 4; ++i) { const float d = t[2 * rg + jj][i] - mw[rg]; q = fmaf(d, d, q); }
+    qw[rg] = sum_lanes_16_32(q);
+  }
+  if (g == 0) {
+#pragma unroll
+    for (int rg = 0; rg < 2; ++rg) *reinterpret_cast<float2*>(part + ((16 * rg + c) * 8 + tile) * 2) = make_float2(mw[rg], qw[rg]);
+  }
+  __syncthreads();
+  const float4 gS[2] = {make_float4(gs[0].x * H_ACT_SCALE, gs[0].y * H_ACT_SCALE, gs[0].z * H_ACT_SCALE, gs[0].w * H_ACT_SCALE),
+                        make_float4(gs[1].x * H_ACT_SCALE, gs[1].y * H_ACT_SCALE, gs[1].z * H_ACT_SCALE, gs[1].w * H_ACT_SCALE)};
+  const float4 bS[2] = {make_float4(bs[0].x * H_ACT_SCALE, bs[0].y * H_ACT_SCALE, bs[0].z * H_ACT_SCALE, bs[0].w * H_ACT_SCALE),
+                        make_float4(bs[1].x * H_ACT_SCALE, bs[1].y * H_ACT_SCALE, bs[1].z * H_ACT_SCALE, bs[1].w * H_ACT_SCALE)};
+#pragma unroll
+  for (int rg = 0; rg < 2; ++rg) {
+    float4 pr[4];
+#pragma unroll
+    for (int j = 0; j < 4; ++j) pr[j] = *reinterpret_cast<const float4*>(part + (16 * rg + c) * 16 + 4 * j);
+    const float mean = (((pr[0].x + pr[0].z) + (pr[1].x + pr[1].z)) + ((pr[2].x + pr[2].z) + (pr[3].x + pr[3].z))) * 0.125f;
+    float m2 = ((pr[0].y + pr[0].w) + (pr[1].y + pr[1].w)) + ((pr[2].y + pr[2].w) + (pr[3].y + pr[3].w));
+    float dd = 0.0f;
+#pragma unroll
+    for (int j = 0; j < 4; ++j) {
+      const float d0 = pr[j].x - mean, d1 = pr[j].z - mean;
+      dd = fmaf(d0, d0, dd); dd = fmaf(d1, d1, dd);
+    }
+    m2 = fmaf(dd, 32.0f, m2);
+    const float rstd = 1.0f / sqrtf(m2 * (1.0f / 256.0f) + 1e-5f * (H_ACT_SCALE * H_ACT_SCALE));
+#pragma unroll
+    for (int jj = 0; jj < 2; ++jj) {
+      float* v = t[2 * rg + jj];
+      v[0] = fmaf((v[0] - mean) * rstd, gS[jj].x, bS[jj].x);
+      v[1] = fmaf((v[1] - mean) * rstd, gS[jj].y, bS[jj].y);
+      v[2] = fmaf((v[2] - mean) * rstd, gS[jj].z, bS[jj].z);
+      v[3] = fmaf((v[3] - mean) * rstd, gS[jj].w, bS[jj].w);
+    }
+    __builtin_amdgcn_sched_barrier(0);
+  }
+}
+
 struct Acc32H;
-template <bool DROP>
+template <bool DROP, bool LNF = false>
 __device__ __forceinline__ void lin_epilogue32(const LinSpec& s, int colbase, const f32x4 (&thi)[4], const f32x4 (&tlo)[4], int lane,
                                                const float4 (&bias4)[2]) {
   const int c = lane & 15, g = lane >> 4;
@@ -919,6 +996,73 @@
     for (int v = 0; v < 4; ++v) {
       t[v][0] = fmaf(rf[v].x, H_ACT_SCALE, t[v][0]); t[v][1] = fmaf(rf[v].y, H_ACT_SCALE, t[v][1]);
       t[v][2] = fmaf(rf[v].z, H_ACT_SCALE, t[v][2]); t[v][3] = fmaf(rf[v].w, H_ACT_SCALE, t[v][3]);
+    }
+  }
+  if constexpr (LNF) {
+    if (s.ln_g != nullptr) {
+      auto plane_ptr = [&](float* base, int v) {
+        const int col = colb + 16 * (v & 1), rloc = 16 * (v >> 1) + c;
+        return reinterpret_cast<char*>(base + rloc * LD2) + (col >> 3) * 32 + (col & 7) * 2;
+      };
+      if (s.ln_flags & E_LN_RES2) {
+#pragma unroll
+        for (int v = 0; v < 4; ++v) {
+          const char* p = plane_ptr(s.ln_aux, v);
+          const uint2 ph = *reinterpret_cast<const uint2*>(p), pl = *reinterpret_cast<const uint2*>(p + 16);
+          const f16x2 h0 = __builtin_bit_cast(f16x2, ph.x), h1 = __builtin_bit_cast(f16x2, ph.y);
+          const f16x2 l0 = __builtin_bit_cast(f16x2, pl.x), l1 = __builtin_bit_cast(f16x2, pl.y);
+          t[v][0] += fmaf((float)l0[0], 1.0f / H_LO_SCALE, (float)h0[0]); t[v][1] += fmaf((float)l0[1], 1.0f / H_LO_SCALE, (float)h0[1]);
+          t[v][2] += fmaf((float)l1[0], 1.0f / H_LO_SCALE, (float)h1[0]); t[v][3] += fmaf((float)l1[1], 1.0f / H_LO_SCALE, (float)h1[1]);
+        }
+      }
+      float4 lng[2], lnb[2], lnpos[4];
+#pragma unroll
+      for (int jj = 0; jj < 2; ++jj) { lng[jj] = ld4(s.ln_g + colb + 16 * jj); lnb[jj] = ld4(s.ln_b + colb + 16 * jj); }
+      if (s.ln_flags & F_LN_XP) {
+#pragma unroll
+        for (int v = 0; v < 4; ++v) {
+          int prow = min(s.m0 + 16 * (v >> 1) + c, s.M - 1);
+          if (s.pos_mod > 0) prow = prow % s.pos_mod;
+          lnpos[v] = ld4(s.pos + (size_t)prow * s.pos_ld + colb + 16 * (v & 1));
+        }
+      }
+      ln_stage32(t, lng, lnb, s.ln_part, colbase >> 5, c, g);
+      if (s.ln_flags & F_LN_RELU) {
+#pragma unroll
+        for (int v = 0; v < 4; ++v)
+#pragma unroll
+          for (int i = 0; i < 4; ++i) t[v][i] = relu_(t[v][i]);
+      }
+#pragma unroll
+      for (int v = 0; v < 4; ++v) {
+        uint2 h, l;
+        split_t2(t[v][0], t[v][1], h.x, l.x);
+        split_t2(t[v][2], t[v][3], h.y, l.y);
+        char* p = plane_ptr(s.dst, v);
+        *reinterpret_cast<uint2*>(p) = h;
+        *reinterpret_cast<uint2*>(p + 16) = l;
+      }
+      if (s.ln_flags & F_LN_XP) {
+#pragma unroll
+        for (int v = 0; v < 4; ++v) {
+          uint2 h, l;
+          split_t2(fmaf(lnpos[v].x, H_ACT_SCALE, t[v][0]), fmaf(lnpos[v].y, H_ACT_SCALE, t[v][1]), h.x, l.x);
+          split_t2(fmaf(lnpos[v].z, H_ACT_SCALE, t[v][2]), fmaf(lnpos[v].w, H_ACT_SCALE, t[v][3]), h.y, l.y);
+          char* p = plane_ptr(s.ln_aux, v);
+          *reinterpret_cast<uint2*>(p) = h;
+          *reinterpret_cast<uint2*>(p + 16) = l;
+        }
+      }
+      if (s.gdst != nullptr) {
+#pragma unroll
+        for (int v = 0; v < 4; ++v) {
+          const int col = colb + 16 * (v & 1), rloc = 16 * (v >> 1) + c;
+          if (s.m0 + rloc >= s.M) continue;
+          const int grow = s.rowg != nullptr ? s.rowg[rloc] : s.m0 + rloc;
+          st4(s.gdst + (size_t)grow * s.gdst_ld + col, make_float4(t[v][0] * US, t[v][1] * US, t[v][2] * US, t[v][3] * US));
+        }
+      }
+      return;
     }
   }
   if (s.dst != nullptr) {
@@ -1090,7 +1234,7 @@
   }
 }
 
-template <bool DROP, bool NB = false, typename SpecFn>
+template <bool DROP, bool NB = false, bool LNF = false, typename SpecFn>
 __device__ __forceinline__ bool linear_step32h(const LinSpec& s, WBuf& w0, bool preloaded, const float* next_first,
                                                SpecFn make_spec, int step_idx) {
   constexpr int NW = 8;
@@ -1157,7 +1301,7 @@
         if (tile * 32 + 32 <= e.N) {
           const f32x4 thi[4] = {acc.hi[0][0], acc.hi[0][1], acc.hi[1][0], acc.hi[1][1]};
           const f32x4 tlo[4] = {acc.lo[0][0], acc.lo[0][1], acc.lo[1][0], acc.lo[1][1]};
-          lin_epilogue32<DROP>(e, tile * 32, thi, tlo, lane, bias4);
+          lin_epilogue32<DROP, LNF>(e, tile * 32, thi, tlo, lane, bias4);
         } else {
           f32x4 y[4];
 #pragma unroll
@@ -1192,10 +1336,10 @@
   return next_first != nullptr;
 }
 
-template <int R, bool DROP, bool SRC2, int MM, bool NB = false, typename SpecFn>
+template <int R, bool DROP, bool SRC2, int MM, bool NB = false, bool LNF = false, typename SpecFn>
 __device__ __forceinline__ bool linear_step(const LinSpec& s, WBuf& w0, bool preloaded,
                                             const float* next_first, SpecFn make_spec, int step_idx) {
-  if constexpr (R == 32) return linear_step32h<DROP, NB>(s, w0, preloaded, next_first, make_spec, step_idx);
+  if constexpr (R == 32) return linear_step32h<DROP, NB, LNF>(s, w0, preloaded, next_first, make_spec, step_idx);
   if constexpr (R == 16 && MM == 1) return linear_step16h<DROP>(s, w0, preloaded, next_first, make_spec, step_idx);
   if constexpr (R == 16) return linear_step16<DROP, SRC2>(s, w0, preloaded, next_first, make_spec, step_idx);
   constexpr int NG = R / 4;
@@ -1353,6 +1497,7 @@
 __device__ __forceinline__ void chain_body(const ChainDev& k, const StepAllT<nw_of(R)>* __restrict__ recs, const int block) {
   constexpr int NW = nw_of(R), NT = NW * 64;
   constexpr bool PL = R == 32;
+  constexpr bool FUSE = fuses_ln32(R, PROG, MM, DROP, MP);
   static_assert((MM == 0 && R <= 16) || (MM == 1 && R >= 16 && PROG != PROG_PROLOGUE), "the f16 two-plane path exists for 16- and 32-row tiles (and is the only one at 32)");
   extern __shared__ __align__(16) unsigned char smem_raw[];
   using Lds = ChainLds<R, rec_cap(PROG)>;
@@ -1538,6 +1683,8 @@
     s.drop_site = 0; s.drop_seed = 0; s.drop_thr = 0; s.drop_scale = 1.0f; s.drop_stride = 0; s.drop_q = 0;
     s.rowg = nullptr; s.gpre = 0; s.cmask = nullptr; s.cscale = 1.0f;
     s.dst_pl = 0; s.res_pl = 0; s.range_flag = nullptr;
+    s.ln_g = nullptr; s.ln_b = nullptr; s.ln_flags = 0; s.ln_aux = nullptr; s.ln_part = nullptr;
+    s.pos = nullptr; s.pos_ld = 0; s.pos_mod = 0;
     return s;
   };
   auto epi_spec = [&](int j) {
@@ -1565,6 +1712,19 @@
     s.gpre = (e.flags & F_GPRE) ? 1 : 0;
     s.dst_pl = PL && e.dst_ld != LDL; s.res_pl = PL && e.res_ld != LDL;
     s.range_flag = MM == 1 ? k.range_status : nullptr;
+    s.ln_g = nullptr; s.ln_b = nullptr; s.ln_flags = 0; s.ln_aux = nullptr; s.ln_part = nullptr;
+    s.pos = nullptr; s.pos_ld = 0; s.pos_mod = 0;
+    if constexpr (FUSE) {
+      if (e.flags & E_LN) {
+        struct LnPair { const float* g; const float* b; };
+        const LnPair lp = load_uniform<LnPair>(*reinterpret_cast<const LnPair*>(&S.recs[j].r.p2));
+        s.ln_g = lp.g; s.ln_b = lp.b;
+        s.ln_flags = e.flags & (F_LN_RELU | F_LN_XP | E_LN_RES2);
+        s.ln_aux = e.aux_off >= 0 ? base + e.aux_off : nullptr;
+        s.ln_part = &S.lnpart.p[0][0][0];
+        s.pos = k.g[G_POS]; s.pos_ld = k.g_ld[G_POS]; s.pos_mod = k.g_mod[G_POS];
+      }
+    }
     if (DROP) {
       if constexpr (PROG == PROG_RADAR_TRAIN) {
         s.drop_site = e.drop_site; s.drop_seed = k.rdrop.seed; s.drop_thr = k.rdrop.thr; s.drop_scale = k.rdrop.scale;
@@ -1624,7 +1784,16 @@
           if (kd == K_LINEAR && (r.flags & F_IFHIT)) skip = !tile_has_hit();
         }
         if (skip) {
-          if (r.res != B_NONE && r.dst != B_NONE) {
+          bool ln_only = false;
+          if constexpr (FUSE) ln_only = r.p2 != nullptr;
+          if (ln_only) {
+            if constexpr (FUSE) {
+              const LinSpec e = epi_spec(idx);
+              const f32x4 z[4] = {f32x4{0.f, 0.f, 0.f, 0.f}, f32x4{0.f, 0.f, 0.f, 0.f}, f32x4{0.f, 0.f, 0.f, 0.f}, f32x4{0.f, 0.f, 0.f, 0.f}};
+              const float4 zb[2] = {make_float4(0.f, 0.f, 0.f, 0.f), make_float4(0.f, 0.f, 0.f, 0.f)};
+              lin_epilogue32<DROP, true>(e, 32 * ((wave - e.woff) & (NW - 1)), z, z, lane, zb);
+            }
+          } else if (r.res != B_NONE && r.dst != B_NONE) {
             const float* rs = buf_ptr(S, r.res); const int rld = buf_ld(r.res);
             float* dd = buf_ptr(S, r.dst);
             for (int row = wave; row < R; row += NW)
@@ -1638,7 +1807,7 @@
 #endif
           if (((wave - s.woff) & (NW - 1)) < (R == 32 ? (s.N + 31) >> 5 : (s.N + 63) >> 6)) {
             const PreRec pr = load_uniform<PreRec>(S.recs[idx].p[wave]);
-            const bool have = linear_step<R, DROP, PROG == PROG_PROLOGUE, MM, MP>(s, w0, pre_idx == idx, pr.first, epi_spec, idx);
+            const bool have = linear_step<R, DROP, PROG == PROG_PROLOGUE, MM, MP, FUSE>(s, w0, pre_idx == idx, pr.first, epi_spec, idx);
             pre_idx = have ? pr.nidx : -1;
           }
         } else if (kd == K_LN) {
@@ -2250,6 +2419,83 @@
 static_assert(chain_lds_bytes<16, PROG_RADAR>() <= 80 * 1024 && chain_lds_bytes<32, PROG_RADAR>() <= 160 * 1024, "radar programs: LDS per workgroup");
 inline int buf_ld_h(int id) { return id == B_A ? LD5 : id == B_L ? LDL : LD2; }
 
+inline bool bufs_overlap(int a, int b) {
+  if (a == B_NONE || b == B_NONE) return false;
+  auto in_a = [](int x) { return x == B_A || x == B_U1 || x == B_U2; };
+  return a == b || ((a == B_A || b == B_A) && in_a(a) && in_a(b));
+}
+inline bool step_touches(const StepRes& m, int buf) {
+  return bufs_overlap(m.src, buf) || bufs_overlap(m.src2, buf) || bufs_overlap(m.dst, buf) || bufs_overlap(m.res, buf);
+}
+template <int NW, class OffFn>
+int fuse_ln32(StepAllT<NW>* out, int total, const ChainK& k, int l0_seq, OffFn off) {
+  auto can_carry = [](const StepRes& r, bool own_gd) {
+    return r.kind == K_LINEAR && r.N == 256 && r.p2 == nullptr && (own_gd || r.gd == nullptr) && r.gt == nullptr &&
+           !(r.flags & (F_WAVE1 | F_GPRE | F_CMASK | F_SKIP_NONEXT)) && r.dst >= B_X && r.dst <= B_U3;
+  };
+  auto carry = [&](StepAllT<NW>& p, const float* g, const float* b, int lnflags, int dst, int aux, bool res2, float* gd) {
+    p.r.p2 = g; p.r.p3 = b;
+    p.r.flags = (short)(p.r.flags | (lnflags & (F_LN_RELU | F_LN_XP)));
+    p.r.dst = (short)dst;
+    if (gd != nullptr) { p.r.gd = gd; p.r.gld = 256; }
+    p.e.flags = (int)p.r.flags | E_LN | (res2 ? E_LN_RES2 : 0);
+    p.e.dst_off = off(dst); p.e.dst_ld = LD2;
+    p.e.aux_off = aux != B_NONE ? off(aux) : -1;
+    p.e.gd = p.r.gd; p.e.gld = p.r.gld;
+  };
+  int n = 0;
+  for (int j = 0; j < total; ++j) {
+    const StepAllT<NW> cur = out[j];
+    const StepRes& c = cur.r;
+    bool gone = false;
+    if (c.kind == K_LN) {
+      const bool xp = (c.flags & F_LN_XP) != 0;
+      int p = n - 1;
+      for (; p >= 0; --p) {
+        const StepRes& m = out[p].r;
+        if (m.kind == K_LINEAR && m.dst == c.src) break;
+        if (m.kind == K_NOP) continue;
+        if (m.kind != K_LINEAR || step_touches(m, c.src) || step_touches(m, c.dst) || step_touches(m, c.src2) ||
+            (xp && step_touches(m, c.res))) { p = -1; break; }
+      }
+      if (p >= 0 && can_carry(out[p].r, false) && (xp || c.res == B_NONE)) {
+        const bool ifhit = (out[p].r.flags & F_IFHIT) != 0;
+        if (c.src2 == B_NONE) {
+          if (!ifhit || ((out[p].r.flags & F_GATE) && out[p].r.res != B_NONE)) {
+            carry(out[p], c.p0, c.p1, c.flags, c.dst, xp ? c.res : B_NONE, false, c.gd);
+            gone = true;
+          }
+        } else if (p == n - 1 && !xp && !ifhit && !step_touches(out[p].r, c.src2)) {
+          bool ready = l0_seq == 1;
+          if (!ready && n >= 2 && can_carry(out[n - 2].r, false) && out[n - 2].r.dst == c.src2 && !(out[n - 2].r.flags & F_IFHIT)) {
+            carry(out[n - 2], c.p2, c.p3, F_LN_RELU, c.src2, B_NONE, false, nullptr);
+            ready = true;
+          }
+          if (ready) {
+            carry(out[p], c.p0, c.p1, 0, c.dst, c.src2, true, c.gd);
+            gone = true;
+          }
+        }
+      }
+      if (!gone && l0_seq == 1 && c.src2 != B_NONE) return -1;
+    }
+    if (gone) { out[n - 1].r.sync = (short)(out[n - 1].r.sync | c.sync); continue; }
+    out[n] = cur;
+    if (l0_seq == 2 && c.kind == K_LINEAR && c.gd != nullptr && c.gd == k.g[G_KV1]) {
+      if (!can_carry(c, true)) return -1;
+      carry(out[n], k.pairs[8].w, k.pairs[8].b, F_LN_RELU, c.dst, B_NONE, false, c.gd);
+    }
+    ++n;
+  }
+  if (n < total) memset(static_cast<void*>(out + n), 0, sizeof(StepAllT<NW>) * (size_t)(total - n));
+  bool open = false;
+  for (int i = 0; i < n; ++i) {
+    if (out[i].e.flags & E_LN) { if (open) return -1; open = true; }
+    if (out[i].r.sync) open = false;
+  }
+  return n;
+}
+
 template <int R, int PROG, int MM = 0>
 void resolve_program(ChainK& k, StepAllT<nw_of(R)>* out) {
   constexpr int NW = nw_of(R);
@@ -2262,7 +2508,7 @@
   if (prog_is_enc_full(PROG) || PROG == PROG_RADAR_ENC_A || PROG == PROG_RADAR_ENC_B)
     while (nsteps > 0 && table[nsteps - 1].kind == K_LINEAR && table[nsteps - 1].wp >= 7 + k.nlayers) --nsteps;
   const int nrep = (prog_is_radar(PROG) || PROG == PROG_RADAR_BWD) ? k.nlayers : 1;
-  const int total = nsteps * nrep;
+  int total = nsteps * nrep;
   memset(out, 0, sizeof(StepAllT<NW>) * rec_cap(PROG));
   for (int idx = 0; idx < total; ++idx) {
     const int rep = idx / nsteps, si = idx - rep * nsteps;
@@ -2362,6 +2608,8 @@
     e.dst_off = lds_off<R, PROG>(r.dst); e.dst_ld = buf_ld_h(r.dst);
     e.res_off = lds_off<R, PROG>(r.res); e.res_ld = buf_ld_h(r.res);
   }
+  if (fuses_ln32(R, PROG, MM, k.drop.thr != 0, PROG == PROG_DECODER && generic_xattn(k)))
+    total = fuse_ln32<NW>(out, total, k, PROG == PROG_DECODER ? k.l0_seq : 0, lds_off<R, PROG>);
   for (int idx = 0; idx < total; ++idx) {
     for (int w = 0; w < NW; ++w) {
       PreRec& pr = out[idx].p[w];
@@ -2419,6 +2667,7 @@
   Recs<rec_cap(PROGB), nw_of(RB)> rb;
   resolve_program<RA, PROG_DECODER, MM>(ka, ra.s);
   resolve_program<RB, PROGB, MM>(kb, rb.s);
+  TC_REQUIRE(ka.total >= 0 && kb.total >= 0, "%s: the record sequence cannot carry its LayerNorms in the linear steps", what);
   const int na = (ka.M + RA - 1) / RA, nb = (kb.M + RB - 1) / RB;
   hipLaunchKernelGGL((chain_dual_kernel<RA, RB, PROGB, MM, PRE, MP>), dim3(na + nb), dim3(nw_of(RA) * 64), lds, s,
                      static_cast<const ChainDev&>(ka), static_cast<const ChainDev&>(kb), na, ra, rb);
@@ -2434,6 +2683,7 @@
   if (const int rc = need_packed16(R, k.w16_delta, what)) return rc;
   Recs<rec_cap(PROG), nw_of(R)> recs;
   resolve_program<R, PROG, MM>(k, recs.s);
+  TC_REQUIRE(k.total >= 0, "%s: the record sequence cannot carry its LayerNorms in the linear steps", what);
   hipLaunchKernelGGL((chain_kernel<R, PROG, DROP, MM, PRE, MP>), dim3((k.M + R - 1) / R), dim3(nw_of(R) * 64), lds, s,
                      static_cast<const ChainDev&>(k), recs);
   return check_launch(what);
@@ -2943,6 +3193,48 @@
 }
 }
 
+namespace {
+__global__ __launch_bounds__(512) void ln_epilogue_selfcheck_kernel(const float* __restrict__ x, const float* __restrict__ gamma,
+                                                                    const float* __restrict__ beta, float* __restrict__ y, int fused) {
+  __shared__ float part[32 * 8 * 2];
+  const int lane = threadIdx.x & 63, wave = threadIdx.x >> 6;
+  const float* xt = x + (size_t)blockIdx.x * 32 * 256;
+  float* yt = y + (size_t)blockIdx.x * 32 * 256;
+  if (fused) {
+    const int c = lane & 15, g = lane >> 4, colb = 32 * wave + 4 * g;
+    float4 gs[2], bs[2];
+#pragma unroll
+    for (int jj = 0; jj < 2; ++jj) { gs[jj] = ld4(gamma + colb + 16 * jj); bs[jj] = ld4(beta + colb + 16 * jj); }
+    float t[4][4];
+#pragma unroll
+    for (int v = 0; v < 4; ++v) {
+      const float4 a = ld4(xt + (16 * (v >> 1) + c) * 256 + colb + 16 * (v & 1));
+      t[v][0] = a.x * H_ACT_SCALE; t[v][1] = a.y * H_ACT_SCALE; t[v][2] = a.z * H_ACT_SCALE; t[v][3] = a.w * H_ACT_SCALE;
+    }
+    ln_stage32(t, gs, bs, part, wave, c, g);
+    constexpr float US = 1.0f / H_ACT_SCALE;
+#pragma unroll
+    for (int v = 0; v < 4; ++v)
+      st4(yt + (16 * (v >> 1) + c) * 256 + colb + 16 * (v & 1), make_float4(t[v][0] * US, t[v][1] * US, t[v][2] * US, t[v][3] * US));
+  } else {
+    const float4 gg = ld4(gamma + 4 * lane), bb = ld4(beta + 4 * lane);
+    float4 v[4];
+#pragma unroll
+    for (int i = 0; i < 4; ++i) v[i] = ld4(xt + (wave + 8 * i) * 256 + 4 * lane);
+    ln_rows<4>(v, gg, bb);
+#pragma unroll
+    for (int i = 0; i < 4; ++i) st4(yt + (wave + 8 * i) * 256 + 4 * lane, v[i]);
+  }
+}
+}
+
+int launch_ln_epilogue_selfcheck(const float* x, const float* gamma, const float* beta, float* y, int n_tiles, int fused, hipStream_t s) {
+  TC_REQUIRE(n_tiles > 0 && x != nullptr && gamma != nullptr && beta != nullptr && y != nullptr && (fused == 0 || fused == 1),
+             "ln_epilogue_selfcheck: bad arguments");
+  hipLaunchKernelGGL(ln_epilogue_selfcheck_kernel, dim3(n_tiles), dim3(512), 0, s, x, gamma, beta, y, fused);
+  return check_launch("ln_epilogue_selfcheck");
+}
+
 int launch_rowops_selfcheck(int n_blocks, unsigned long long seed, unsigned long long* mismatches, hipStream_t s) {
   TC_REQUIRE(n_blocks > 0 && mismatches != nullptr, "rowops_selfcheck: bad arguments");
   hipLaunchKernelGGL(rowops_selfcheck_kernel, dim3(n_blocks), dim3(256), 0, s, seed, mismatches);
diff --git a/transcar_amd/csrc/head.hip b/transcar_amd/csrc/head.hip
--- a/transcar_amd/csrc/head.hip
+++ b/transcar_amd/csrc/head.hip
@@ -709,6 +709,11 @@
   return launch_rowops_selfcheck(n_blocks, seed, mismatches, as_stream(stream));
 }
 
+int tc_ln_epilogue_selfcheck(const float* x, const float* gamma, const float* beta, float* y, int n_tiles, int fused,
+                             tc_stream_t stream) {
+  return launch_ln_epilogue_selfcheck(x, gamma, beta, y, n_tiles, fused, as_stream(stream));
+}
+
 size_t tc_box_decode_workspace_bytes(int B, int Q, int num_classes) {
   return box_decode_ws_bytes(B, Q, num_classes);
 }
diff --git a/transcar_amd/csrc/kernels.hpp b/transcar_amd/csrc/kernels.hpp
--- a/transcar_amd/csrc/kernels.hpp
+++ b/transcar_amd/csrc/kernels.hpp
@@ -175,6 +175,7 @@
 
 int launch_gate_selfcheck(int n_radii, unsigned long long seed, unsigned long long* mismatches, hipStream_t s);
 int launch_rowops_selfcheck(int n_blocks, unsigned long long seed, unsigned long long* mismatches, hipStream_t s);
+int launch_ln_epilogue_selfcheck(const float* x, const float* gamma, const float* beta, float* y, int n_tiles, int fused, hipStream_t s);
 
 inline bool heads_ok(int num_heads) { return num_heads == 4 || num_heads == 8 || num_heads == 16; }
 int launch_self_attn_core(const float* q, const float* k, int ld, const float* vt, int ldt,
```
